# Kuntz-Lab/interactive-rate-tendons

Hardware: AMD Instinct MI355X
Metric: FK+collision checks/sec (3-tendon, 256^3 voxel env) (higher is better)
Workload: dtype f64

## Files before the change

include/tendon_hip.h:

```cpp
#ifndef TENDON_HIP_H
#define TENDON_HIP_H

#include <stddef.h>
#include <stdint.h>

#ifdef __cplusplus
extern "C" {
#endif

#define TR_MAX_TENDONS 8
#define TR_MAX_COEF    8

typedef enum {
  TR_OK                = 0,
  TR_ERR_INVALID_ARG   = 1,
  TR_ERR_OUT_OF_RANGE  = 2,
  TR_ERR_DOMAIN        = 3,
  TR_ERR_LENGTH        = 4,
  TR_ERR_RUNTIME       = 5,
  TR_ERR_HIP           = 6,
  TR_ERR_UNSUPPORTED   = 7
} tr_status;

typedef struct {
// ... 358 lines not shown
int tr_roadmap_state_query_profile(tr_roadmap *rm, double out[4]);

int tr_roadmap_ik_batch_loaded(tr_roadmap *rm, const tr_space_params *sp, const tr_tip_query_params *params, const tr_tip_connect_params *connect,
                               const tr_shoot_params *shoot, const tr_edge_loads *loads, const double *requests, int64_t n, double *controls,
                               double *tips, double *error, int32_t *neighbor_vertex, int32_t *ik_vertex, int32_t *outcome,
                               double *last_valid_t, double *vu0, int64_t *counts);
int tr_roadmap_solve_tips_loaded(tr_roadmap *rm, const tr_space_params *sp, const tr_tip_query_params *params, const tr_tip_connect_params *connect,
                                 const tr_shoot_params *shoot, const tr_edge_loads *loads, const int32_t *starts, const double *requests, int64_t n,
                                 int32_t n_threads, double *controls, double *tips, double *error, int32_t *neighbor_vertex, int32_t *ik_vertex,
                                 int32_t *outcome, double *last_valid_t, double *vu0, int64_t *counts, int32_t *status, double *cost,
                                 int64_t *path_offsets, tr_roadmap_stats *stats);
int tr_roadmap_set_tips_loaded(tr_roadmap *rm, const tr_shoot_params *shoot, const tr_edge_loads *loads, const uint64_t *present_bits);

int tr_knn_edges(tr_ctx *ctx, const double *states, int64_t n, int32_t k, double max_distance, int32_t *edges,
                 int64_t capacity, int64_t *n_edges);
int tr_knn_edges_dev(tr_ctx *ctx, const double *d_states, int64_t n, int32_t k, double max_distance, int32_t *d_edges,
                     int64_t capacity, int64_t *n_edges);
int tr_validate_edges_indexed_dev(tr_ctx *ctx, const tr_space_params *sp, const double *d_states, int64_t n_states,
                                  const int32_t *d_edges, int64_t n_edges, uint64_t *d_valid_bits, int32_t *d_n_fk,
                                  int64_t *n_domain_errors);
int tr_signature_words(const tr_ctx *ctx);
int tr_sample_valid_vertices_sig_dev(tr_ctx *ctx, uint64_t seed, uint64_t first_candidate, const double *lo, const double *hi,
                                     int64_t n_want, int64_t max_candidates, double *d_states, double *d_tips, int64_t *d_index,
                                     uint32_t *d_sig, int64_t *n_accepted, int64_t *n_tried, void *stream);
int tr_validate_candidates_sig_dev(tr_ctx *ctx, uint64_t seed, uint64_t first, int64_t count, const double *lo, const double *hi,
                                   uint64_t *d_valid_bits, double *d_tips, uint32_t *d_sig, void *stream);
int tr_validate_edges_indexed_sig_dev(tr_ctx *ctx, const tr_space_params *sp, const double *d_states, int64_t n_states,
                                      const uint32_t *d_vertex_sig, const int32_t *d_edges, int64_t n_edges,
                                      uint64_t *d_valid_bits, int32_t *d_n_fk, int64_t *n_domain_errors);

int tr_signature_packed_words(const tr_ctx *ctx);
int tr_pack_signatures_dev(tr_ctx *ctx, const uint32_t *d_sig, int64_t n_rows, uint32_t *d_packed, int64_t *n_uncodable, void *stream);
int tr_unpack_signatures_dev(tr_ctx *ctx, const uint32_t *d_packed, int64_t n_rows, uint32_t *d_sig, void *stream);

int tr_knn_range(tr_ctx *ctx, const double *states, int64_t n, int64_t first_query, int64_t n_queries, int32_t k,
                 double max_distance, int32_t *idx, double *dist);
int tr_knn_table_edges(tr_ctx *ctx, const int32_t *idx, int64_t n, int32_t k, int32_t *edges, int64_t capacity, int64_t *n_edges);
int tr_knn_range_dev(tr_ctx *ctx, const double *d_states, int64_t n, int64_t first_query, int64_t n_queries, int32_t k,
                     double max_distance, int32_t *d_idx);
int tr_knn_table_edges_dev(tr_ctx *ctx, const int32_t *d_idx, int64_t n, int32_t k, int32_t *d_edges, int64_t capacity,
                           int64_t *n_edges);

int tr_kstar_k(const tr_ctx *ctx, int64_t n_milestones);


#define TR_PROFILE_SLOTS 6
int tr_profile_begin(tr_ctx *ctx);
int tr_profile_read(tr_ctx *ctx, int64_t launches[TR_PROFILE_SLOTS], double total_ms[TR_PROFILE_SLOTS]);
int tr_profile_end(tr_ctx *ctx);

int tr_set_debug(tr_ctx *ctx, uint32_t bits);

int tr_edge_schedule_last(const tr_ctx *ctx, uint32_t stats[4]);


#ifdef __cplusplus
}
#endif
#endif
```

interactive-rate-tendons_amd/_lib.py:

```python
import ctypes as C
import os
import subprocess

_PKG = os.path.dirname(os.path.abspath(__file__))
_ROOT = os.path.dirname(_PKG)
LIB_PATH = os.environ.get("TENDON_HIP_LIB") or os.path.join(_PKG, "libtendon_hip.so")
SRC_DIR = os.path.join(_PKG, "csrc")
HEADER = os.path.join(_ROOT, "include", "tendon_hip.h")

TR_OK, TR_ERR_INVALID_ARG, TR_ERR_OUT_OF_RANGE, TR_ERR_DOMAIN, TR_ERR_LENGTH, TR_ERR_RUNTIME, \
    TR_ERR_HIP, TR_ERR_UNSUPPORTED = range(8)

TR_FLAG_CONVERGED, TR_FLAG_LENGTH_OK, TR_FLAG_NO_SELFCOL, TR_FLAG_NO_VOXCOL, TR_FLAG_DOMAIN = 1, 2, 4, 8, 16
TR_CHECKER_BACKBONE, TR_CHECKER_SPHERES = 0, 1
TR_PROFILE_SLOTS = 6
PROFILE_SLOT_NAMES = ("fk_rk4_batch", "backbone_voxel_sweep", "cached_blocks_vs_grid", "edge_helpers", "fk_sweep_fused", "fk_verdict")

ABI_SYMBOLS = (
    "tr_create", "tr_destroy", "tr_last_error", "tr_state_size", "tr_num_points", "tr_device",
    "tr_home_lengths", "tr_set_grid", "tr_set_checker", "tr_grid_add_spheres", "tr_grid_add_capsules", "tr_grid_remove_interior", "tr_grid_dilate",
    "tr_grid_dilate_sphere", "tr_get_grid", "tr_reserve", "tr_reserve_edges", "tr_fk_batch", "tr_fk_batch_dev", "tr_fk_batch_retraction_dev",
    "tr_validate_shapes_retraction_dev",
    "tr_validate_batch", "tr_validate_batch_dev", "tr_validate_shapes_dev", "tr_validate_edges", "tr_validate_edges_indexed", "tr_validate_edges_last_valid",
    "tr_validate_edges_discrete",
    "tr_check_cached", "tr_check_cached_dev", "tr_check_cached_subset_dev", "tr_state_layout", "tr_space_weights", "tr_kstar_k",
    "tr_roadmap_create", "tr_roadmap_destroy", "tr_roadmap_last_error", "tr_roadmap_set_caches", "tr_roadmap_set_caches_dev", "tr_roadmap_prepare", "tr_roadmap_clear_validity",
    "tr_roadmap_revalidate", "tr_roadmap_get_validity", "tr_roadmap_set_validity", "tr_roadmap_solve", "tr_roadmap_fetch_paths", "tr_roadmap_search_stats", "tr_roadmap_profile", "tr_roadmap_release_search_state", "tr_roadmap_reserve_search_state", "tr_roadmap_search_state_bytes", "tr_roadmap_search_sweeps", "tr_voxelize_batch", "tr_voxelize_edges", "tr_voxelize_edges_indexed", "tr_connect_edges_indexed", "tr_voxelize_fetch", "tr_voxelize_fetch_dev", "tr_voxelize_count", "tr_knn", "tr_knn_range", "tr_knn_table_edges", "tr_knn_edges", "tr_knn_edges_dev", "tr_knn_range_dev", "tr_knn_table_edges_dev", "tr_validate_edges_indexed_dev", "tr_signature_words", "tr_signature_packed_words", "tr_pack_signatures_dev", "tr_unpack_signatures_dev", "tr_validate_candidates_sig_dev", "tr_validate_edges_indexed_sig_dev", "tr_profile_begin", "tr_profile_read", "tr_profile_end",
    "tr_set_debug", "tr_edge_schedule_last",
    "tr_candidate_states", "tr_candidate_states_dev", "tr_validate_candidates_dev", "tr_compact_rows_dev",
    "tr_sample_valid_vertices", "tr_sample_valid_vertices_dev", "tr_sample_valid_vertices_sig_dev",
    "tr_fk_tips", "tr_fk_tips_dev", "tr_tip_jacobian", "tr_tip_jacobian_dev", "tr_ik_batch", "tr_ik_batch_dev",
    "tr_roadmap_set_tips", "tr_roadmap_nearest_tips", "tr_roadmap_nearest_tips_dev", "tr_roadmap_ik_batch", "tr_roadmap_solve_tips",
    "tr_roadmap_tip_query_profile",
    "tr_roadmap_nearest_states", "tr_roadmap_nearest_states_dev", "tr_roadmap_ik_batch_connect", "tr_roadmap_solve_tips_connect",
    "tr_roadmap_tip_connect_stats",
    "tr_fk_loaded_batch", "tr_fk_loaded_batch_dev", "tr_fk_loaded_batch_retraction_dev", "tr_set_loaded_retraction",
    "tr_validate_edges_loaded", "tr_validate_edges_loaded_indexed", "tr_edges_loaded_vertex_strains", "tr_edges_loaded_last",
    "tr_sample_valid_vertices_loaded", "tr_sample_valid_vertices_loaded_dev", "tr_voxelize_batch_loaded",
    "tr_voxelize_edges_loaded_indexed", "tr_connect_edges_loaded_indexed",
    "tr_ik_loaded_batch", "tr_ik_loaded_batch_dev",
    "tr_tip_jacobian_loaded", "tr_tip_jacobian_loaded_dev",
    "tr_fk_loaded_tips", "tr_fk_loaded_tips_dev",
    "tr_roadmap_ik_batch_loaded", "tr_roadmap_solve_tips_loaded", "tr_roadmap_set_tips_loaded",
    "tr_set_load_profile", "tr_clear_load_profile", "tr_get_load_profile",
    "tr_roadmap_attach_states", "tr_roadmap_attach_states_dev", "tr_roadmap_solve_seeded", "tr_roadmap_solve_states",
    "tr_roadmap_state_query_profile",
)


class TrRobotDesc(C.Structure):
    _fields_ = [
        ("r", C.c_double),
        ("L", C.c_double), ("dL", C.c_double), ("ro", C.c_double), ("ri", C.c_double),
        ("E", C.c_double), ("nu", C.c_double),
        ("n_tendons", C.c_int32), ("n_a", C.c_int32), ("n_m", C.c_int32),
        ("C", C.POINTER(C.c_double)), ("D", C.POINTER(C.c_double)),
        ("max_tension", C.POINTER(C.c_double)), ("min_length", C.POINTER(C.c_double)),
        ("max_length", C.POINTER(C.c_double)),
        ("enable_rotation", C.c_int32), ("enable_retraction", C.c_int32),
        ("residual_threshold", C.c_double),
    ]


class TrSpaceParams(C.Structure):
    _fields_ = [("min_tension_change", C.c_double), ("min_rotation_change", C.c_double),
                ("min_retraction_change", C.c_double)]


class TrIkParams(C.Structure):
    _fields_ = [("max_iters", C.c_int32), ("mu_init", C.c_double), ("stop_threshold_JT_err_inf", C.c_double),
                ("stop_threshold_Dp", C.c_double), ("stop_threshold_err", C.c_double), ("finite_difference_delta", C.c_double)]


class TrShootParams(C.Structure):
    _fields_ = [("max_iters", C.c_int32), ("mu_init", C.c_double), ("stop_threshold_JT_err_inf", C.c_double),
                ("stop_threshold_Dp", C.c_double), ("finite_difference_delta", C.c_double)]


TR_LOAD_FRAME_BASE, TR_LOAD_FRAME_WORLD = 0, 1


# ... 276 lines not shown
    L.tr_fk_loaded_batch_dev.argtypes = [vp, shp, vp, i64, i64, vp, i64, vp, i64, vp, vp, vp, vp, vp, vp, vp, vp, vp, vp, vp, vp, vp, vp, P(i64), vp]
    L.tr_set_loaded_retraction.argtypes = [vp, C.c_int]
    L.tr_fk_loaded_batch_retraction_dev.argtypes = [vp, shp, vp, i64, i64, vp, i64, vp, i64, vp, vp, vp, vp, vp, vp, vp, vp, vp, vp, vp, vp, vp, vp, vp, P(i64), vp]
    elp = P(TrEdgeLoads)
    L.tr_validate_edges_loaded.argtypes = [vp, P(TrSpaceParams), shp, elp, dp, dp, i64, P(C.c_uint64), dp, i32p, P(i64), P(i64), P(i64)]
    L.tr_validate_edges_loaded_indexed.argtypes = [vp, P(TrSpaceParams), shp, elp, dp, i64, i32p, i64, P(C.c_uint64), i32p, P(i64), P(i64), P(i64)]
    L.tr_edges_loaded_vertex_strains.argtypes = [vp, i64, dp]
    L.tr_edges_loaded_last.argtypes = [vp, P(i64)]
    L.tr_sample_valid_vertices_loaded.argtypes = [vp, shp, elp, u64, u64, dp, dp, i64, i64, dp, dp, P(i64), dp, P(i64), P(i64), P(i64), P(i64)]
    L.tr_sample_valid_vertices_loaded_dev.argtypes = [vp, shp, elp, u64, u64, dp, dp, i64, i64, vp, vp, vp, vp, P(i64), P(i64), P(i64), P(i64), vp]
    L.tr_voxelize_batch_loaded.argtypes = [vp, shp, elp, dp, i64, P(i64), P(C.c_uint64), dp, P(i64), P(i64)]
    L.tr_voxelize_edges_loaded_indexed.argtypes = [vp, P(TrSpaceParams), shp, elp, dp, i64, i32p, i64, P(i64), P(C.c_uint64), i32p, P(i64), P(i64)]
    L.tr_connect_edges_loaded_indexed.argtypes = L.tr_voxelize_edges_loaded_indexed.argtypes
    L.tr_ik_loaded_batch.argtypes = [vp, P(TrIkParams), shp, elp, dp, i64, dp, i64, dp, dp, dp, dp, dp, dp, i32p, i32p, dp, P(C.c_uint8), P(i64)]
    L.tr_ik_loaded_batch_dev.argtypes = [vp, P(TrIkParams), shp, elp, vp, i64, vp, i64, dp, dp, vp, vp, vp, vp, vp, vp, vp, vp, P(i64), vp]
    L.tr_tip_jacobian_loaded.argtypes = [vp, shp, elp, dp, i64, C.c_double, dp, dp, dp, dp, dp, dp, P(C.c_uint8), dp, P(i64), P(i64)]
    L.tr_tip_jacobian_loaded_dev.argtypes = [vp, shp, elp, vp, i64, C.c_double, vp, vp, vp, vp, vp, vp, vp, vp, vp, P(i64), vp]
    tqp = P(TrTipQueryParams)
    L.tr_roadmap_set_tips.argtypes = [vp, dp, P(u64)]
    L.tr_roadmap_nearest_tips.argtypes = [vp, dp, i64, C.c_int32, i32p, dp]
    L.tr_roadmap_nearest_tips_dev.argtypes = [vp, vp, i64, C.c_int32, vp, vp]
    L.tr_roadmap_ik_batch.argtypes = [vp, P(TrSpaceParams), tqp, dp, i64, dp, dp, dp, i32p, i32p, dp]
    L.tr_roadmap_solve_tips.argtypes = [vp, P(TrSpaceParams), tqp, i32p, dp, i64, C.c_int32, dp, dp, dp, i32p, i32p, dp, i32p, dp, P(i64),
                                        P(TrRoadmapStats)]
    L.tr_roadmap_tip_query_profile.argtypes = [vp, dp]
    tcp = P(TrTipConnectParams)
    L.tr_roadmap_nearest_states.argtypes = [vp, dp, i64, C.c_int32, C.c_double, i32p, dp]
    L.tr_roadmap_nearest_states_dev.argtypes = [vp, vp, i64, C.c_int32, C.c_double, vp, vp]
    L.tr_roadmap_ik_batch_connect.argtypes = [vp, P(TrSpaceParams), tqp, tcp, dp, i64, dp, dp, dp, i32p, i32p, i32p, dp]
    L.tr_roadmap_solve_tips_connect.argtypes = [vp, P(TrSpaceParams), tqp, tcp, i32p, dp, i64, C.c_int32, dp, dp, dp, i32p, i32p, i32p, dp, i32p,
                                                dp, P(i64), P(TrRoadmapStats)]
    L.tr_roadmap_tip_connect_stats.argtypes = [vp, P(i64)]
    L.tr_fk_loaded_tips.argtypes = [vp, shp, dp, i64, dp, i64, dp, i64, dp, dp, P(C.c_uint8), dp, P(i64)]
    L.tr_fk_loaded_tips_dev.argtypes = [vp, shp, vp, i64, vp, i64, vp, i64, vp, vp, vp, vp, P(i64), vp]
    L.tr_roadmap_ik_batch_loaded.argtypes = [vp, P(TrSpaceParams), tqp, tcp, shp, elp, dp, i64, dp, dp, dp, i32p, i32p, i32p, dp, dp, P(i64)]
    L.tr_roadmap_solve_tips_loaded.argtypes = [vp, P(TrSpaceParams), tqp, tcp, shp, elp, i32p, dp, i64, C.c_int32, dp, dp, dp, i32p, i32p, i32p,
                                               dp, dp, P(i64), i32p, dp, P(i64), P(TrRoadmapStats)]
    L.tr_roadmap_set_tips_loaded.argtypes = [vp, shp, elp, P(u64)]
    atp, u8p = P(TrAttachParams), P(C.c_uint8)
    L.tr_roadmap_attach_states.argtypes = [vp, P(TrSpaceParams), atp, C.c_int32, dp, i64, u8p, i32p, dp, u8p, i32p, P(i64)]
    L.tr_roadmap_attach_states_dev.argtypes = [vp, P(TrSpaceParams), atp, C.c_int32, vp, i64, vp, vp, vp, vp, vp, P(i64)]
    L.tr_roadmap_solve_seeded.argtypes = [vp, i64, P(i64), i32p, dp, P(i64), i32p, dp, dp, C.c_int32, i32p, dp, i32p, i32p, P(i64), P(TrRoadmapStats)]
    L.tr_roadmap_solve_states.argtypes = [vp, P(TrSpaceParams), atp, dp, dp, i64, C.c_int32, i32p, dp, i32p, i32p, u8p, i32p, i32p, P(i64),
                                          P(TrRoadmapStats)]
    L.tr_roadmap_state_query_profile.argtypes = [vp, dp]
    L.tr_set_load_profile.argtypes = [vp, i64, dp, dp]
    L.tr_clear_load_profile.argtypes = [vp]
    L.tr_get_load_profile.argtypes = [vp, dp, i64, P(i64)]
    L.tr_profile_begin.argtypes = [vp]
    L.tr_profile_read.argtypes = [vp, P(i64), dp]
    L.tr_profile_end.argtypes = [vp]
    L.tr_set_debug.argtypes = [vp, C.c_uint32]
    L.tr_edge_schedule_last.argtypes = [vp, P(C.c_uint32)]
    _lib = L
    return L


def check(ctx, status):
    if status == TR_OK:
        return
    msg = lib().tr_last_error(ctx)
    msg = msg.decode() if msg else "status %d" % status
    raise _EXC.get(status, TendonHipError)(msg)
```

interactive-rate-tendons_amd/csrc/edge_queue_kernel.hpp:

```cpp
#pragma once
#include "verdict_kernel.hpp"
#define TRK_EDGE_DEVICE_ONLY
#include "edge_kernel.hpp"

namespace trk {

__device__ __forceinline__ uint32_t eq_load(const uint32_t *p) { return __hip_atomic_load(p, __ATOMIC_RELAXED, __HIP_MEMORY_SCOPE_AGENT); }
__device__ __forceinline__ void eq_wait_vm() { asm volatile("s_waitcnt vmcnt(0)" ::: "memory"); }
__device__ __forceinline__ void eq_release() {
  eq_wait_vm();
  __builtin_amdgcn_fence(__ATOMIC_RELEASE, "agent");
  eq_wait_vm();
}
__device__ __forceinline__ void eq_acquire() {
  __builtin_amdgcn_fence(__ATOMIC_ACQUIRE, "agent");
  eq_wait_vm();
}
__device__ __forceinline__ int eq_bcast(int v) { return __builtin_amdgcn_readfirstlane(v); }
struct EqClock {
  unsigned long long t;
  __device__ __forceinline__ void start() { t = wall_clock64(); }
  __device__ __forceinline__ void lap(uint32_t *ctl, int word) {
    const unsigned long long n = wall_clock64();
    if (threadIdx.x == 0) __hip_atomic_fetch_add((unsigned long long *)(ctl + word), n - t, __ATOMIC_RELAXED, __HIP_MEMORY_SCOPE_AGENT);
// ... 77 lines not shown
    if (n > 0) { pos = eq_bcast(r_pos); return true; }
    d = (uint32_t)eq_bcast((int)d); t = (uint32_t)eq_bcast((int)t);
    if (d + t != seen) { seen = d + t; idle = 0; }
    else if (++idle > (1u << 19)) {
      if (lane == 0) __hip_atomic_fetch_or(ctl + EQ_FLAGS, EQF_STUCK, __ATOMIC_RELAXED, __HIP_MEMORY_SCOPE_AGENT);
      return false;
    }
    __builtin_amdgcn_s_sleep(127);
    if (idle > 16) __builtin_amdgcn_s_sleep(127);
    if (idle > 256) { __builtin_amdgcn_s_sleep(127); __builtin_amdgcn_s_sleep(127); }
  }
}

template <int N, bool ROT, class Form = TableRouting>
__global__ __launch_bounds__(64, (N <= TRK_VERDICT_TWO_WAVE_MAXN ? 2 : 1)) void fk_edge_queue(
    RobotK K, const double *__restrict__ tab, const StepK *__restrict__ steps, int nsteps,
    const VerdictArgs *__restrict__ va, const EdgeQueueArgs *__restrict__ qa, const FusedSweepArgs *__restrict__ sa) {
  const int lane = threadIdx.x;
  EqClock clk;
  clk.start();
#ifdef TRK_EQ_TRACE
  int tr_round = 0;
#endif
  for (;;) {
    int zero = 0;
    asm volatile("" : "+s"(zero));
    const EdgeQueueArgs &q = qa[zero];
    int h = 0, cnt = 0;
    if (!eq_claim(q, h, cnt)) break;
    clk.lap(q.ctl, EQ_T_CLAIM);
    const bool live = lane < cnt;
    const int slot = h + lane;
    int e_lane = -1;
    {
      bool bail = false;
      if (live) {
        const uint32_t *flag = (const uint32_t *)q.sample_edge + slot;
        unsigned spins = 0;
        while ((e_lane = (int)eq_load(flag)) < 0) {
          if (eq_load(q.ctl + EQ_FLAGS) != 0u) { bail = true; break; }
          if (++spins > (1u << 22)) {
            __hip_atomic_fetch_or(q.ctl + EQ_FLAGS, EQF_STUCK, __ATOMIC_RELAXED, __HIP_MEMORY_SCOPE_AGENT);
            bail = true; break;
          }
          __builtin_amdgcn_s_sleep(8);
        }
      }
      if (__any(bail)) break;
    }
    eq_acquire();
    clk.lap(q.ctl, EQ_T_READY);

    PointSweep<false, true> ps;
    ps.va = va;
    ps.dn_prev = 0.0f; ps.sph_state = 0u;
    ps.qhead = 0; ps.qcount = 0; ps.active = false;
    ps.P = va->P; ps.CH = va->CH; ps.NM = va->NM; ps.Kl = (ps.P - 1 + ps.CH - 1) / ps.CH; ps.ms_next = 0; ps.ms_k = 0;
    ps.sigst.init(); ps.sig_row_of = -1; ps.sig_first_row = 0; ps.sig_row0 = h; ps.sig_cnt = cnt;
    __syncthreads();
    VL_U(VLay<true>::HIT + lane) = 0u; VL_U(VLay<true>::INPREV + lane) = 0u; VL_F(VLay<true>::DIST + lane) = 0.0f;
    __syncthreads();
    const int S = K.state_size;
    const double *st_eff = q.states + ((int64_t)h - (int64_t)blockIdx.x * 64) * S;
    const int64_t n_eff = (int64_t)blockIdx.x * 64 + cnt;
    {
      const int sb = eq_stash_base(ps.NM);
      VL_I(sb + lane) = e_lane;
      if (lane == 0) { VL_I(sb + 64) = h; VL_I(sb + 65) = cnt; VL_U(sb + 66) = (uint32_t)clk.t; VL_U(sb + 67) = (uint32_t)(clk.t >> 32); }
    }
    FkLane<N> fl_;
    {
      FkOut out{nullptr, nullptr, nullptr, nullptr, nullptr, nullptr, nullptr, nullptr, nullptr, nullptr};
      fk_uniform_body<N, ROT, false, false, Form>(st_eff, n_eff, 0, K, tab, steps, nsteps, out, ps, nullptr, &fl_);
    }
    ps.template sig_finish<false>();
    ps.finish();
    while (ps.qcount > 0) ps.flush();
    __syncthreads();
    LaneVerdict lv;
    int e2, h2, cnt2;
    {
      const VerdictArgs a = *va;
      const int sb = eq_stash_base(a.NM);
      e2 = VL_I(sb + lane); h2 = VL_I(sb + 64); cnt2 = VL_I(sb + 65);
      clk.t = (unsigned long long)VL_U(sb + 66) | ((unsigned long long)VL_U(sb + 67) << 32);
      lv = verdict_decide<N, false, true>(a, fl_, lane < cnt2);
    }
    const bool live2 = lane < cnt2;
    int zero2 = 0;
    asm volatile("" : "+s"(zero2));
    const EdgeQueueArgs &q2 = qa[zero2];
#ifdef TRK_EQ_TRACE
    const uint32_t tr_start = (uint32_t)clk.t;
    const unsigned long long tr_w0 = wall_clock64(), tr_c0 = (unsigned long long)clock64();
    { float x = (float)lane; for (int i = 0; i < 2000; i++) x = __builtin_fmaf(x, 1.0000001f, 0.5f); if (x == 12345.678f) asm volatile("s_nop 0"); }
    const unsigned long long tr_w1 = wall_clock64(), tr_c1 = (unsigned long long)clock64();
    const uint32_t tr_mhz = tr_w1 > tr_w0 ? (uint32_t)((tr_c1 - tr_c0) * 100ull / (tr_w1 - tr_w0)) : 0u;
#endif
    clk.lap(q2.ctl, EQ_T_FK);
#ifdef TRK_EQ_TRACE
    const uint32_t tr_fk = (uint32_t)clk.t;
#endif
    if (__any(lv.pending)) {
      __syncthreads();
      const double *st2 = q2.states + ((int64_t)h2 - (int64_t)blockIdx.x * 64) * K.state_size;
      const int64_t n2 = (int64_t)blockIdx.x * 64 + cnt2;
      fk_uniform_body<N, ROT, false, false, Form>(st2, n2, q2.fb_ld, K, tab, steps, nsteps, q2.fb_out, NoPointHook(), nullptr, nullptr);
      __syncthreads();
      const FusedSweepArgs fa = *sa;
      bool exact = false;
      sweep_body<false>(q2.fb_in, n2, q2.fb_ld, fa.P, fa.CH, fa.NM, K, fa.g, fa.grid, fa.near_grid, 1, fa.debug, nullptr, nullptr, nullptr, &exact);
      __syncthreads();
      const uint32_t npend = (uint32_t)__popcll(__ballot(lv.pending));
// ... 167 lines not shown
```

interactive-rate-tendons_amd/csrc/fk_inst.hip:

```cpp
#include "fk_launch.hpp"
#include "fk_kernel.hpp"
#if TRK_INST_KIND == 1
#include "fk_retract_kernel.hpp"
#elif TRK_INST_KIND == 2
#include "fused_kernel.hpp"
#elif TRK_INST_KIND == 3
#include "verdict_kernel.hpp"
#elif TRK_INST_KIND == 4
#define TRK_WITH_RETRACT_VERDICT
#include "fk_retract_kernel.hpp"
#include "verdict_kernel.hpp"
#elif TRK_INST_KIND == 5
#include "edge_queue_kernel.hpp"
#elif TRK_INST_KIND == 6 || TRK_INST_KIND == 7
#define TRK_LOADED_WITH_INTEGRATOR
#include "fk_loaded_kernel.hpp"
#elif TRK_INST_KIND == 8
#include "fk_loaded_retract_kernel.hpp"
#endif

namespace trk {

using HelixForm = std::conditional_t<(TRK_INST_N <= TRK_K1_TWO_WAVE_MAXN), UniformHelix, TableRouting>;
[[maybe_unused]] static bool helix_form(const RobotK &K) { return TRK_INST_N <= TRK_K1_TWO_WAVE_MAXN && K.routing_form == TRK_ROUTING_HELIX; }
// ... 44 lines not shown
static void go(const FkLaunch &a, const LoadedIn &in) {
  const unsigned grid = (unsigned)((a.n + 63) / 64);
  hipLaunchKernelGGL((fk_loaded_profile<TRK_INST_N, ROT, WR>), dim3(grid), dim3(64), 0, a.stream, a.d_states, a.n, a.ld, a.K,
                     a.d_tab, a.d_steps, a.n_steps, a.out, in);
}
template <> void launch_fk_loaded_profile<TRK_INST_N>(const FkLaunch &a, const LoadedIn &in) {
  if (a.rotation) { if (a.write_R) go<true, true>(a, in); else go<true, false>(a, in); }
  else            { if (a.write_R) go<false, true>(a, in); else go<false, false>(a, in); }
}
#elif TRK_INST_KIND == 8
template <bool ROT, bool WR>
static void go(const FkLaunch &a, const LoadedIn &in) {
  const unsigned grid = (unsigned)((a.n + 63) / 64);
  hipLaunchKernelGGL((fk_loaded_retract<TRK_INST_N, ROT, WR>), dim3(grid), dim3(64), 0, a.stream, a.d_states, a.n, a.ld, a.K, a.d_poly,
                     a.d_tab, a.d_steps, a.n_steps, a.k_first, a.d_tgrid, a.d_hl, a.out, in);
}
template <> void launch_fk_loaded_retract<TRK_INST_N>(const FkLaunch &a, const LoadedIn &in) {
  if (a.rotation) { if (a.write_R) go<true, true>(a, in); else go<true, false>(a, in); }
  else            { if (a.write_R) go<false, true>(a, in); else go<false, false>(a, in); }
}
template <> void launch_shoot_start_retract<TRK_INST_N>(const FkLaunch &a, const double *guess, double *vu) {
  const unsigned grid = (unsigned)((a.n + 63) / 64);
  hipLaunchKernelGGL((shoot_start_retract<TRK_INST_N>), dim3(grid), dim3(64), 0, a.stream, a.d_states, a.n, a.K, a.d_poly, guess, vu);
}
#elif TRK_INST_KIND == 4
template <bool ROT, bool SPH, bool SIG>
static void go(const FkLaunch &a, const VerdictArgs *va, size_t lds) {
  const unsigned grid = (unsigned)((a.n + 63) / 64);
  const RetractHandoff ho{a.d_handoff, a.handoff_ld};
  hipLaunchKernelGGL((fk_retract_prologue<TRK_INST_N, ROT>), dim3(grid), dim3(64), 0, a.stream, a.d_states, a.n, a.K, a.d_poly, a.d_tab, a.d_steps,
                     a.n_steps, a.k_first, a.d_tgrid, a.d_hl, a.d_perm, ho);
  hipLaunchKernelGGL((fk_verdict_retract<TRK_INST_N, ROT, SPH, SIG>), dim3(grid), dim3(64), lds, a.stream, a.d_states, a.n, a.K, a.d_poly,
                     a.d_tab, a.d_steps, a.n_steps, a.k_first, a.d_tgrid, a.d_hl, a.out.tips, va, ho);
}
template <bool SPH, bool SIG>
static void go_rot(const FkLaunch &a, const VerdictArgs *va, size_t lds) {
  if (a.rotation) go<true, SPH, SIG>(a, va, lds); else go<false, SPH, SIG>(a, va, lds);
}
template <> void launch_fk_verdict_retract<TRK_INST_N>(const FkLaunch &a, const VerdictArgs *va, size_t lds, bool spheres, bool with_sig) {
  if (spheres) { if (with_sig) go_rot<true, true>(a, va, lds); else go_rot<true, false>(a, va, lds); }
  else         { if (with_sig) go_rot<false, true>(a, va, lds); else go_rot<false, false>(a, va, lds); }
}
template <bool ROT>
static void go_list(const FkLaunch &a, const FusedSweepArgs *sweep, size_t lds, const int32_t *list, const uint32_t *count) {
  const unsigned grid = (unsigned)((a.n + 63) / 64);
  hipLaunchKernelGGL((fk_sweep_retract_list<TRK_INST_N, ROT>), dim3(grid), dim3(64), lds, a.stream, a.d_states, a.n, a.ld, a.K,
                     a.d_poly, a.d_tab, a.d_steps, a.n_steps, a.k_first, a.d_tgrid, a.d_hl, a.out, sweep, list, count);
}
template <> void launch_fk_sweep_retract_list<TRK_INST_N>(const FkLaunch &a, const FusedSweepArgs *sweep, size_t lds, const int32_t *list,
                                                          const uint32_t *count) {
  if (a.rotation) go_list<true>(a, sweep, lds, list, count); else go_list<false>(a, sweep, lds, list, count);
}
#elif TRK_INST_KIND == 3
template <bool ROT, bool SPH, bool SIG, class Form>
static void go(const FkLaunch &a, const VerdictArgs *va, size_t lds) {
  const unsigned grid = (unsigned)((a.n + 63) / 64);
  hipLaunchKernelGGL((fk_verdict<TRK_INST_N, ROT, SPH, SIG, Form>), dim3(grid), dim3(64), lds, a.stream, a.d_states, a.n, a.K, a.d_tab, a.d_steps,
                     a.n_steps, a.out.tips, va);
}
template <bool SPH, bool SIG>
static void go_rot(const FkLaunch &a, const VerdictArgs *va, size_t lds) {
  if (helix_form(a.K)) { if (a.rotation) go<true, SPH, SIG, HelixForm>(a, va, lds); else go<false, SPH, SIG, HelixForm>(a, va, lds); }
  else                 { if (a.rotation) go<true, SPH, SIG, TableRouting>(a, va, lds); else go<false, SPH, SIG, TableRouting>(a, va, lds); }
}
template <> void launch_fk_verdict<TRK_INST_N>(const FkLaunch &a, const VerdictArgs *va, size_t lds, bool spheres, bool with_sig) {
  if (spheres) { if (with_sig) go_rot<true, true>(a, va, lds); else go_rot<true, false>(a, va, lds); }
  else         { if (with_sig) go_rot<false, true>(a, va, lds); else go_rot<false, false>(a, va, lds); }
}
#elif TRK_INST_KIND == 2
template <bool ROT, class Form>
static void go_list(const FkLaunch &a, const FusedSweepArgs *sweep, size_t lds, const int32_t *list, const uint32_t *count) {
  const unsigned grid = (unsigned)((a.n + 63) / 64);
  hipLaunchKernelGGL((fk_sweep_fused_list<TRK_INST_N, ROT, Form>), dim3(grid), dim3(64), lds, a.stream, a.d_states, a.n, a.ld, a.K,
                     a.d_tab, a.d_steps, a.n_steps, a.out, sweep, list, count);
}
template <> void launch_fk_sweep_fused_list<TRK_INST_N>(const FkLaunch &a, const FusedSweepArgs *sweep, size_t lds, const int32_t *list,
                                                        const uint32_t *count) {
  if (helix_form(a.K)) { if (a.rotation) go_list<true, HelixForm>(a, sweep, lds, list, count); else go_list<false, HelixForm>(a, sweep, lds, list, count); }
  else                 { if (a.rotation) go_list<true, TableRouting>(a, sweep, lds, list, count); else go_list<false, TableRouting>(a, sweep, lds, list, count); }
}
template <bool ROT, class Form>
static void go(const FkLaunch &a, const FusedSweepArgs *sweep, size_t lds) {
  const unsigned grid = (unsigned)((a.n + 63) / 64);
  hipLaunchKernelGGL((fk_sweep_fused<TRK_INST_N, ROT, Form>), dim3(grid), dim3(64), lds, a.stream, a.d_states, a.n, a.ld, a.K,
                     a.d_tab, a.d_steps, a.n_steps, a.out, sweep);
}
template <> void launch_fk_sweep_fused<TRK_INST_N>(const FkLaunch &a, const FusedSweepArgs *sweep, size_t lds) {
  if (helix_form(a.K)) { if (a.rotation) go<true, HelixForm>(a, sweep, lds); else go<false, HelixForm>(a, sweep, lds); }
  else                 { if (a.rotation) go<true, TableRouting>(a, sweep, lds); else go<false, TableRouting>(a, sweep, lds); }
}
#else
#if TRK_INST_KIND == 1
template <bool ROT, bool WR>
static void go(const FkLaunch &a) {
  const unsigned grid = (unsigned)((a.n + 63) / 64);
  hipLaunchKernelGGL((fk_rk4_batch_retract<TRK_INST_N, ROT, WR>), dim3(grid), dim3(64), 0, a.stream, a.d_states, a.n, a.ld, a.K,
                     a.d_poly, a.d_tab, a.d_steps, a.n_steps, a.k_first, a.d_tgrid, a.d_hl, a.out, a.d_perm, a.d_wave_k_begin);
}
template <> void launch_fk_retract<TRK_INST_N>(const FkLaunch &a) {
#else
template <bool ROT, bool WR>
static void go(const FkLaunch &a) {
  const unsigned grid = (unsigned)((a.n + 63) / 64);
  if (helix_form(a.K))
    hipLaunchKernelGGL((fk_rk4_batch_uniform<TRK_INST_N, ROT, WR, HelixForm>), dim3(grid), dim3(64), 0, a.stream, a.d_states, a.n, a.ld, a.K,
                       a.d_tab, a.d_steps, a.n_steps, a.out);
  else
    hipLaunchKernelGGL((fk_rk4_batch_uniform<TRK_INST_N, ROT, WR>), dim3(grid), dim3(64), 0, a.stream, a.d_states, a.n, a.ld, a.K,
                       a.d_tab, a.d_steps, a.n_steps, a.out);
}
template <> void launch_fk_uniform<TRK_INST_N>(const FkLaunch &a) {
#endif
  if (a.rotation) { if (a.write_R) go<true, true>(a); else go<true, false>(a); }
  else            { if (a.write_R) go<false, true>(a); else go<false, false>(a); }
}
#endif

}
```

interactive-rate-tendons_amd/csrc/fk_kernel.hpp:

```cpp
#pragma once
#include <type_traits>
#include <hip/hip_runtime.h>
#include "tr_types.hpp"

namespace trk {

#ifndef TRK_NEWTON_STEPS
#define TRK_NEWTON_STEPS 1
#endif
__device__ __forceinline__ double fast_rcp(double x) {
  double y = __builtin_amdgcn_rcp(x);
  double e = __builtin_fma(-x, y, 1.0);
  y = __builtin_fma(e, y, y);
#if TRK_NEWTON_STEPS > 1
  e = __builtin_fma(-x, y, 1.0);
  y = __builtin_fma(e, y, y);
#endif
  return y;
}
__device__ __forceinline__ double fast_rsqrt(double x) {
  double y = __builtin_amdgcn_rsq(x);
  double hx = 0.5 * x;
  double t = __builtin_fma(-hx * y, y, 0.5);
  y = __builtin_fma(y, t, y);
// ... 281 lines not shown
#pragma clang fp contract(fast)
  const double hh = h * 0.5;
  const double b1 = h * (1.0 / 6.0), b2 = h * (1.0 / 3.0);
  double aR[9], av[3], au[3];
#pragma unroll
  for (int q = 0; q < 3; q++) { av[q] = v[q]; au[q] = u[q]; }
  double sR[9], sv[3], su[3], qs[3], qm[3];
#pragma unroll
  for (int q = 0; q < 9; q++) sR[q] = R[q];
#pragma unroll
  for (int q = 0; q < 3; q++) { sv[q] = v[q]; su[q] = u[q]; }
#pragma unroll
  for (int st = 0; st < 4; st++) {
    double ts = (st == 0) ? t : ((st == 3) ? t + h : t + hh);
    asm volatile("" : "+v"(ts) : "v"(sv[0]), "v"(su[0]));
    const double bw = (st == 0 || st == 3) ? b1 : b2;
    const double aw = (st == 2) ? h : hh;
    double dv[3], du[3], sd[N];
    strain_rates_routed<N>(sv, su, tau, [&](int j, double (&r6)[6]) { route(ts, j, r6); }, K, dv, du, sd, stage_load(sR));
    position_quadrature(st, sR, sv, b1, qs, qm, p);
    {
      const double v2 = __builtin_fma(sv[2], sv[2], __builtin_fma(sv[1], sv[1], sv[0] * sv[0]));
      Lb += bw * (v2 * fast_rsqrt(v2));
    }
#pragma unroll
    for (int j = 0; j < N; j++) Li[j] += bw * sd[j];
    double dR[9];
    frame_rate(st, sR, su, dR, aR);
#pragma unroll
    for (int q = 0; q < 3; q++) { av[q] += bw * dv[q]; au[q] += bw * du[q]; }
    if (st < 3) {
#pragma unroll
      for (int q = 0; q < 9; q++) sR[q] = R[q] + aw * dR[q];
#pragma unroll
      for (int q = 0; q < 3; q++) { sv[q] = v[q] + aw * dv[q]; su[q] = u[q] + aw * du[q]; }
    }
  }
#pragma unroll
  for (int q = 0; q < 9; q++) R[q] = __builtin_fma(b1, aR[q], R[q]);
#pragma unroll
  for (int q = 0; q < 3; q++) { v[q] = av[q]; u[q] = au[q]; }
}


template <int N>
struct FkLane {
  bool converged;
  double Li[N];
  double tip[3];
};

struct NoPointHook {
  __device__ __forceinline__ void begin(bool) const {}
  __device__ __forceinline__ void operator()(int, double, double, double) const {}
  __device__ __forceinline__ void tip_point(int, bool, bool, double, double, double, bool = true) const {}
};

template <class H, class = void> struct HookLiInLds { static constexpr int from = 1 << 30; };
template <class H> struct HookLiInLds<H, std::void_t<decltype(H::kLiInLdsFrom)>> { static constexpr int from = H::kLiInLdsFrom; };
template <class OnPoint> __host__ __device__ constexpr bool li_in_lds(int N) {
  return N >= HookLiInLds<std::remove_cv_t<std::remove_reference_t<OnPoint>>>::from && N <= 4;
}

template <int N, bool ROT, bool WRITE_R, bool WANT_L = true, class Form = TableRouting, class OnPoint = NoPointHook>
__device__ __forceinline__ void fk_uniform_body(
    const double *__restrict__ states, int64_t n, int64_t ld, const RobotK &K,
    const double *__restrict__ tab, const StepK *__restrict__ steps, int nsteps, const FkOut &out,
    OnPoint &&on_point = NoPointHook(), const int32_t *__restrict__ row_map = nullptr, FkLane<N> *lane_out = nullptr) {
#pragma clang fp contract(fast)
  const int64_t i = (int64_t)blockIdx.x * 64 + threadIdx.x;
  const bool live = i < n;
  const int64_t il = live ? i : (n - 1);
  const int64_t ic = row_map ? (int64_t)row_map[il] : il;
  const int S = K.state_size;
  double tau[N];
#pragma unroll
  for (int j = 0; j < N; j++) tau[j] = states[ic * S + j];
  constexpr bool kLiLds = li_in_lds<OnPoint>(N);
  double *li_lds = nullptr;
  if constexpr (kLiLds) {
    __shared__ double li_lds_store[N * 64];
    li_lds = li_lds_store;
#pragma unroll
    for (int j = 0; j < N; j++) li_lds[j * 64 + threadIdx.x] = 0.0;
  }
  double rc = 1.0, rs = 0.0, r22 = 1.0;
  if (ROT) {
    const double th = states[ic * S + N];
    rs = sin(th); rc = cos(th);
    r22 = (1.0 - rc) + rc;
  }

  double v[3], u[3];
  bool conv;
  initial_bending<N>(tau, tab, K, v, u, conv);
  on_point.begin(conv && live);

  double R[9] = {1, 0, 0, 0, 1, 0, 0, 0, 1};
  double p[3] = {0, 0, 0};
  double Lb = 0;
  double Li[N];
#pragma unroll
  for (int j = 0; j < N; j++) Li[j] = 0;

  auto store_point = [&](int j) {
    const int64_t o = (int64_t)j * ld + i;
    double x = p[0], y = p[1], z = p[2];
    if (ROT) { const double x2 = __builtin_fma(rc, x, -(rs * y)), y2 = __builtin_fma(rs, x, rc * y); x = x2; y = y2; z = r22 * z; }
    on_point(j, x, y, z);
    if (!live) return;
    if (out.px) { out.px[o] = x; out.py[o] = y; out.pz[o] = z; }
    if (WRITE_R) {
      const int64_t PS = (int64_t)K.n_points * ld;
#pragma unroll
      for (int c = 0; c < 3; c++) {
        double a = R[c * 3 + 0], b = R[c * 3 + 1], cc = R[c * 3 + 2];
        if (ROT) { const double a2 = rc * a - rs * b, b2 = rs * a + rc * b; a = a2; b = b2; cc = r22 * cc; }
        out.R[(c * 3 + 0) * PS + o] = a; out.R[(c * 3 + 1) * PS + o] = b; out.R[(c * 3 + 2) * PS + o] = cc;
      }
    }
  };
  store_point(0);

  for (int k = 0; k < nsteps; k++) {
    const double h = steps[k].h;
    const int obs = steps[k].obs;
    const double *__restrict__ rt = tab + (size_t)(1 + 3 * k) * (N * 6);
    const double hh = h * 0.5;
    const double b1 = h * (1.0 / 6.0), b2 = h * (1.0 / 3.0);
    double aR[9], av[3], au[3];
#pragma unroll
    for (int q = 0; q < 3; q++) { av[q] = v[q]; au[q] = u[q]; }
    double sR[9], sv[3], su[3];
    double qs[3], qm[3];
#pragma unroll
    for (int q = 0; q < 9; q++) sR[q] = R[q];
#pragma unroll
    for (int q = 0; q < 3; q++) { sv[q] = v[q]; su[q] = u[q]; }

#pragma unroll
    for (int st = 0; st < 4; st++) {
      const double *__restrict__ ri = rt + (st == 0 ? 0 : (st == 3 ? 2 : 1)) * (N * 6);
      const double bw = (st == 0 || st == 3) ? b1 : b2;
      const double aw = (st == 2) ? h : hh;
      double dv[3], du[3], sd[N];
      strain_rates<N, NoLoad, Form>(sv, su, tau, ri, K, dv, du, sd);
      position_quadrature(st, sR, sv, b1, qs, qm, p);
      if (WANT_L && out.L) {
        const double v2 = __builtin_fma(sv[2], sv[2], __builtin_fma(sv[1], sv[1], sv[0] * sv[0]));
        Lb += bw * (v2 * fast_rsqrt(v2));
      }
      if constexpr (kLiLds) {
#pragma unroll
        for (int j = 0; j < N; j++) li_lds[j * 64 + threadIdx.x] += bw * sd[j];
      } else {
#pragma unroll
        for (int j = 0; j < N; j++) Li[j] += bw * sd[j];
      }
      double dR[9];
      frame_rate(st, sR, su, dR, aR);
#pragma unroll
      for (int q = 0; q < 3; q++) { av[q] += bw * dv[q]; au[q] += bw * du[q]; }
      if (st < 3) {
#pragma unroll
        for (int q = 0; q < 9; q++) sR[q] = R[q] + aw * dR[q];
#pragma unroll
        for (int q = 0; q < 3; q++) { sv[q] = v[q] + aw * dv[q]; su[q] = u[q] + aw * du[q]; }
      }
    }
#pragma unroll
    for (int q = 0; q < 9; q++) R[q] = __builtin_fma(b1, aR[q], R[q]);
#pragma unroll
    for (int q = 0; q < 3; q++) { v[q] = av[q]; u[q] = au[q]; }
    if (obs >= 0) store_point(obs);
  }

  if constexpr (kLiLds) {
#pragma unroll
    for (int j = 0; j < N; j++) Li[j] = li_lds[j * 64 + threadIdx.x];
  }
  if (live) {
    if (out.L) out.L[i] = Lb;
    if (out.Li) {
#pragma unroll
      for (int j = 0; j < N; j++) out.Li[(int64_t)j * ld + i] = Li[j];
    }
    if (out.converged) out.converged[i] = conv ? 1 : 0;
    if (out.n_points) out.n_points[i] = K.n_points;
    if (out.tips) {
      double x = p[0], y = p[1], z = p[2];
      if (ROT) { const double x2 = __builtin_fma(rc, x, -(rs * y)), y2 = __builtin_fma(rs, x, rc * y); x = x2; y = y2; z = r22 * z; }
      out.tips[3 * i + 0] = x; out.tips[3 * i + 1] = y; out.tips[3 * i + 2] = z;
    }
  }
  if (lane_out) {
    lane_out->converged = conv;
#pragma unroll
    for (int j = 0; j < N; j++) lane_out->Li[j] = Li[j];
    double x = p[0], y = p[1], z = p[2];
    if (ROT) { const double x2 = __builtin_fma(rc, x, -(rs * y)), y2 = __builtin_fma(rs, x, rc * y); x = x2; y = y2; z = r22 * z; }
    lane_out->tip[0] = x; lane_out->tip[1] = y; lane_out->tip[2] = z;
  }
}

template <int N, bool ROT, bool WRITE_R, class Form = TableRouting>
__global__ __launch_bounds__(64, (N <= TRK_K1_TWO_WAVE_MAXN ? 2 : 1)) void fk_rk4_batch_uniform(
    const double *__restrict__ states, int64_t n, int64_t ld, RobotK K,
    const double *__restrict__ tab, const StepK *__restrict__ steps, int nsteps, FkOut out) {
  fk_uniform_body<N, ROT, WRITE_R, true, Form>(states, n, ld, K, tab, steps, nsteps, out);
}

}
```

interactive-rate-tendons_amd/csrc/fk_launch.hpp:

```cpp
#pragma once
#include <hip/hip_runtime.h>
#include "tr_types.hpp"

namespace trk {

struct FkLaunch {
  const double *d_states; int64_t n, ld;
  RobotK K;
  bool rotation, write_R;
  const double *d_tab; const StepK *d_steps; int n_steps;
  const PolyK *d_poly; int k_first; const double *d_tgrid, *d_hl;
  FkOut out;
  hipStream_t stream;
  double *d_handoff = nullptr; int64_t handoff_ld = 0; const int32_t *d_perm = nullptr;
  const int32_t *d_wave_k_begin = nullptr;
};

struct LoadedIn {
  const double *wrench; int64_t wrench_ld;
  const double *dist; int64_t dist_ld;
  const double *vu;
  const int32_t *list;
  int32_t Q;
  const double *tip_route;
  double *res; int64_t ldr;
  double *vu_tip;
  const double *weights = nullptr;
};

struct FusedSweepArgs;
struct VerdictArgs;
struct EdgeQueueArgs;
template <int N> void launch_fk_uniform(const FkLaunch &a);
template <int N> void launch_fk_sweep_fused(const FkLaunch &a, const FusedSweepArgs *sweep, size_t lds);
template <int N> void launch_fk_sweep_fused_list(const FkLaunch &a, const FusedSweepArgs *sweep, size_t lds, const int32_t *list,
                                                 const uint32_t *count);
template <int N> void launch_fk_verdict(const FkLaunch &a, const VerdictArgs *va, size_t lds, bool spheres, bool with_sig);
template <int N> void launch_fk_retract(const FkLaunch &a);
template <int N> void launch_fk_verdict_retract(const FkLaunch &a, const VerdictArgs *va, size_t lds, bool spheres, bool with_sig);
template <int N> void launch_fk_sweep_retract_list(const FkLaunch &a, const FusedSweepArgs *sweep, size_t lds, const int32_t *list,
                                                   const uint32_t *count);

template <int N> void launch_fk_edge_queue(const FkLaunch &a, const VerdictArgs *va, size_t lds, const EdgeQueueArgs *qa,
                                           const FusedSweepArgs *sweep, unsigned waves);
template <int N> int fk_edge_queue_waves_per_cu(const RobotK &K, size_t lds);

template <int N> void launch_fk_loaded(const FkLaunch &a, const LoadedIn &in);
template <int N> void launch_fk_loaded_profile(const FkLaunch &a, const LoadedIn &in);
template <int N> void launch_shoot_start(const FkLaunch &a, const double *guess, double *vu);
template <int N> void launch_fk_loaded_retract(const FkLaunch &a, const LoadedIn &in);
template <int N> void launch_shoot_start_retract(const FkLaunch &a, const double *guess, double *vu);

#define TRK_DECL_FK(N) template <> void launch_fk_uniform<N>(const FkLaunch &); template <> void launch_fk_retract<N>(const FkLaunch &); \
  template <> void launch_fk_loaded<N>(const FkLaunch &, const LoadedIn &); template <> void launch_fk_loaded_profile<N>(const FkLaunch &, const LoadedIn &); \
  template <> void launch_shoot_start<N>(const FkLaunch &, const double *, double *); \
  template <> void launch_fk_loaded_retract<N>(const FkLaunch &, const LoadedIn &); \
  template <> void launch_shoot_start_retract<N>(const FkLaunch &, const double *, double *); \
  template <> void launch_fk_sweep_fused<N>(const FkLaunch &, const FusedSweepArgs *, size_t); \
  template <> void launch_fk_sweep_fused_list<N>(const FkLaunch &, const FusedSweepArgs *, size_t, const int32_t *, const uint32_t *); \
  template <> void launch_fk_verdict<N>(const FkLaunch &, const VerdictArgs *, size_t, bool, bool); \
  template <> void launch_fk_verdict_retract<N>(const FkLaunch &, const VerdictArgs *, size_t, bool, bool); \
  template <> void launch_fk_sweep_retract_list<N>(const FkLaunch &, const FusedSweepArgs *, size_t, const int32_t *, const uint32_t *); \
  template <> void launch_fk_edge_queue<N>(const FkLaunch &, const VerdictArgs *, size_t, const EdgeQueueArgs *, const FusedSweepArgs *, unsigned); \
  template <> int fk_edge_queue_waves_per_cu<N>(const RobotK &, size_t);
TRK_DECL_FK(1) TRK_DECL_FK(2) TRK_DECL_FK(3) TRK_DECL_FK(4) TRK_DECL_FK(5) TRK_DECL_FK(6) TRK_DECL_FK(7) TRK_DECL_FK(8)
#undef TRK_DECL_FK

}
```

interactive-rate-tendons_amd/csrc/sweep_kernel.hpp:

```cpp
#pragma once
#include <hip/hip_runtime.h>
#include "tr_types.hpp"

#ifndef TRK_K2_PF
#define TRK_K2_PF 4
#endif

namespace trk {

struct V3 { double x, y, z; };

__device__ __forceinline__ double dot3(const V3 &a, const V3 &b) {
#pragma clang fp contract(off)
  return a.x * b.x + a.y * b.y + a.z * b.z;
}

__device__ __forceinline__ bool segment_aabox_intersect(const V3 &A, const V3 &B, const GridK &g) {
#pragma clang fp contract(off)
  const V3 AB = {B.x - A.x, B.y - A.y, B.z - A.z};
  const double len = sqrt(dot3(AB, AB)) / 2;
  const V3 U = {AB.x / (2 * len), AB.y / (2 * len), AB.z / (2 * len)};
  const V3 Ua = {fabs(U.x), fabs(U.y), fabs(U.z)};
  const V3 P = {(A.x + B.x) / 2 - (g.xmax + g.xmin) / 2, (A.y + B.y) / 2 - (g.ymax + g.ymin) / 2,
                (A.z + B.z) / 2 - (g.zmax + g.zmin) / 2};
// ... 201 lines not shown
  const double tx = A.x - g.xmin, ty = A.y - g.ymin, tz = A.z - g.zmin;
  const double qx = tx * g.inv_dx, qy = ty * g.inv_dy, qz = tz * g.inv_dz;
  int cx = (int)qx, cy = (int)qy, cz = (int)qz;
  const double fx = qx - (double)cx, fy = qy - (double)cy, fz = qz - (double)cz;
  const double lo = 1e-9, hi = 1.0 - 1e-9;
  if (!(fx > lo && fx < hi && fy > lo && fy < hi && fz > lo && fz < hi)) {
    cx = (int)(long)(tx / g.dx); cy = (int)(long)(ty / g.dy); cz = (int)(long)(tz / g.dz);
  }
  return ((uint32_t)cx & 1023u) | (((uint32_t)cy & 1023u) << 10) | (((uint32_t)cz & 1023u) << 20);
}

#ifndef TRK_SIG_FLUSH_UNROLL
#define TRK_SIG_FLUSH_UNROLL 1
#endif
constexpr int SIG_T = 8, SIG_LDS_STRIDE = 72, SIG_LDS_WORDS = SIG_T * SIG_LDS_STRIDE;
struct SigStage {
  int cur, mask;
  __device__ __forceinline__ void init() { cur = -1; mask = 0; }
  template <class Word>
  __device__ __forceinline__ void flush(Word &&W, uint32_t *__restrict__ sig, int64_t stride, int row_of, int first_row) {
    if (cur < 0) return;
    __syncthreads();
    const int lane = threadIdx.x, w = lane & (SIG_T - 1), sub = lane >> 3;
    const int j = cur * SIG_T + w;
#pragma unroll TRK_SIG_FLUSH_UNROLL
    for (int it = 0; it < 8; it++) {
      const int r = it * 8 + sub;
      const int ro = __shfl(row_of, r, 64), fr = __shfl(first_row, r, 64);
      const uint32_t v = W(w * SIG_LDS_STRIDE + r);
      if (((mask >> w) & 1) && ro >= 0 && j >= fr) sig[(int64_t)ro * stride + j] = v;
    }
    __syncthreads();
    cur = -1; mask = 0;
  }
  template <class Word>
  __device__ __forceinline__ void put(Word &&W, uint32_t *__restrict__ sig, int64_t stride, int row_of, int first_row, int row, bool on,
                                      uint32_t value) {
    const int tile = row >> 3;
    if (tile != cur) { flush(W, sig, stride, row_of, first_row); cur = tile; }
    if (on) W((row & (SIG_T - 1)) * SIG_LDS_STRIDE + (int)threadIdx.x) = value;
    mask |= 1 << (row & (SIG_T - 1));
  }
};

struct SignatureHook {
  static constexpr int kLiInLdsFrom = 3;
  const FusedSweepArgs *sa;
  int64_t n;
  bool any;
  SigStage st;
  __device__ __forceinline__ static uint32_t &word(int i) { extern __shared__ float lds[]; return ((uint32_t *)lds)[i]; }
  __device__ __forceinline__ int row_of() const { const int64_t i = (int64_t)blockIdx.x * 64 + threadIdx.x; return i < n ? (int)i : -1; }
  __device__ __forceinline__ void begin(bool) const {}
  __device__ __forceinline__ void operator()(int j, double x, double y, double z) {
    if (!any) return;
    int zero = 0;
    asm volatile("" : "+s"(zero));
    const FusedSweepArgs &a = sa[zero];
    st.put([](int i) -> uint32_t & { return word(i); }, a.sig, a.sig_stride, row_of(), 0, j, true, cell_signature(x, y, z, a.g));
  }
  __device__ __forceinline__ void finish() {
    if (!any) return;
    st.flush([](int i) -> uint32_t & { return word(i); }, sa->sig, sa->sig_stride, row_of(), 0);
  }
};

__device__ __forceinline__ bool exact_self_collision(const SweepIn &in, int64_t ic, int64_t ld, int P, int np,
                                                     bool act, double hmax, double r, bool brute) {
#pragma clang fp contract(off)
  const double consider = 3.0 * r;
  const double rsum = r + r;
  const double h_eff = hmax * (1.0 + 1e-9) + 1e-300;
  const double inv_h = 1.0 / h_eff;
  bool selfhit = false;
  act = act && np > 2;
  for (int a = 0; a < P - 3; ++a) {
    if (!__any(act && a < np - 3)) break;
    const bool act_a = act && a < np - 3;
    const int64_t oa = (int64_t)a * ld + ic;
    V3 pa = {0, 0, 0}, pa1 = {0, 0, 0};
    double acc_a1 = 0;
    if (act_a) {
      pa = V3{in.px[oa], in.py[oa], in.pz[oa]};
      pa1 = V3{in.px[oa + ld], in.py[oa + ld], in.pz[oa + ld]};
      acc_a1 = in.acc[oa + ld];
    }
    int b = a + 2;
    while (b < P - 1) {
      const bool act_b = act_a && !selfhit && b < np - 1;
      if (!__any(act_b)) break;
      int skip = 0x7fffffff;
      if (act_b) {
        const int64_t ob = (int64_t)b * ld + ic;
        const V3 pb = {in.px[ob], in.py[ob], in.pz[ob]};
        skip = 1;
        bool need_exact = true;
        if (!brute) {
          const V3 d = {pa.x - pb.x, pa.y - pb.y, pa.z - pb.z};
          const double D = sqrt(dot3(d, d));
          const double slack = D - rsum - 2.0 * h_eff - 1e-9 * (1.0 + D);
          if (slack > 0.0) {
            need_exact = false;
            const double m = slack * inv_h * (1.0 - 1e-9);
            skip = m > 1.0 ? (m < 1e6 ? (int)m : 1000000) : 1;
          }
        }
        if (need_exact) {
// ... 411 lines not shown
```

interactive-rate-tendons_amd/csrc/tendon_hip.hip:

```cpp
#include <hip/hip_runtime.h>
#include <sched.h>

#include <algorithm>
#include <cfloat>
#include <cmath>
#include <cstdio>
#include <cstdlib>
#include <cstring>
#include <functional>
#include <initializer_list>
#include <chrono>
#include <thread>
#include <ctime>
#include <limits>
#include <mutex>
#include <string>
#include <vector>

#include "../../include/tendon_hip.h"
#include "tr_types.hpp"
#include "fk_launch.hpp"
#include "fk_lin_launch.hpp"
#include "sweep_kernel.hpp"
#include "sphere_kernel.hpp"
// ... 73 lines not shown
    for (T **f : fields) if (const int rc = alloc(c, f, count)) return rc;
    return 0;
  }
  void release() {
    for (void *q : held) (void)hipFree(q);
    held.clear();
  }
};

struct RoundCount {
  tr_ctx *c = nullptr;
  uint32_t *d = nullptr, *h = nullptr;
  int reserve(tr_ctx *ctx, DevOwner &own);
  int zero(int slot, hipStream_t s);
  int read(int slot, hipStream_t s, int64_t &active);
  void release() { if (h) (void)hipHostFree(h); d = h = nullptr; }
};

}

struct tr_ctx {
  std::recursive_mutex mu;
  int device = 0;
  std::string err;
  RobotK K{};
  std::vector<double> C, D, max_tension;
  std::vector<double> t;
  std::vector<StepK> steps;
  std::vector<double> step_t;
  double *d_tab = nullptr;
  StepK *d_steps = nullptr;
  PolyK *d_poly = nullptr;
  double *d_tgrid = nullptr;
  double *d_hl = nullptr;
  int k_first = 0;
  bool has_grid = false;
  GridK G{};
  uint64_t *d_grid = nullptr;
  uint64_t *d_near = nullptr;
  uint32_t n_blocks = 0;
  int checker = TR_CHECKER_BACKBONE;
  float *d_sph_near = nullptr, *d_sph_tmp = nullptr;
  bool sph_near_valid = false;
  uint64_t *d_envw[2] = {nullptr, nullptr};
  uint32_t envw_blocks = 0;
  Workspace ws;
  EdgeDev edge;
  trk::MergeScratch merge;
  int64_t max_chunk = 1 << 20;
  int64_t edge_pool_max = 1 << 22;
  int64_t edge_slots_max = 1 << 24;
  int64_t edge_slots_now = 0;
  double ch_scale = 2.0;
  int64_t k1_round = 1 << 17;
  int fuse = 2;
  int64_t fb_cap = 1 << 17;
  struct RetractOrder {
    uint32_t *keys[2] = {nullptr, nullptr}; int32_t *vals[2] = {nullptr, nullptr}; int64_t cap = 0;
    int32_t *kbegin = nullptr;
    double *handoff = nullptr; int64_t handoff_cap = 0;
    trk::MergeScratch ms;
  };
  static constexpr int kMaxLanes = edge_plan::kMaxLanes;
  struct EdgeLaneDev {
    hipStream_t stream = nullptr;
    uint32_t *hc = nullptr;
    uint32_t *counters = nullptr;
    int32_t *fb_list = nullptr; uint32_t *fb_count = nullptr; int64_t fb_list_cap = 0;
    RetractOrder ro;
  } lane[kMaxLanes];
  int edge_lanes = kMaxLanes;
  bool edge_lanes_fixed = false;
  bool edge_kernels_loaded = false;
  bool edge_queue = true;
  bool edge_queue_forced = false;
  int edge_queue_waves = 0;
  uint32_t edge_queue_last[4] = {0, 0, 0, 0};
  double edge_rate_seen = 0.0;
  bool edge_lane_guess_forced = false;
  double edge_lane_guess = 6.0;
  int64_t retract_sort_min = kRetractSortMin;
  bool rows_one_step = false;
  bool retract_wave_start = true;
  struct VerdictRing {
    static constexpr int kSlots = 16;
    trk::VerdictArgs *d_slots = nullptr, *h_slots = nullptr;
    hipEvent_t ev[kSlots];
    bool used[kSlots] = {};
    int next = 0;
  } vring;
  struct FusedRing {
    static constexpr int kSlots = 16;
    trk::FusedSweepArgs *d_slots = nullptr, *h_slots = nullptr;
    hipEvent_t ev[kSlots];
    bool used[kSlots] = {};
    int next = 0;
  } fused;
  struct KnnScratch { void *p[13] = {}; size_t cap[13] = {}; } knn;
  struct VoxStore { uint32_t *ids = nullptr; uint64_t *masks = nullptr; int64_t cap = 0, n = 0; } vstore;
  uint32_t *d_vids = nullptr; uint64_t *d_vmasks = nullptr; int32_t *d_vcounts = nullptr;
  uint64_t *d_vbits = nullptr;
  int64_t vox_cap = 0;
  int32_t *d_item_src = nullptr, *d_item_edge = nullptr; int64_t vox_items_cap = 0;
  struct Pipe {
    bool ready = false;
    int64_t chunk = 0;
// ... 514 lines not shown
  a.P = ctx->K.n_points; a.debug = ctx->debug;
  a.g = ctx->G; a.grid = ctx->d_grid; a.near_grid = ctx->d_near; a.valid_bits = d_bits; a.flags = d_flags;
  {
    const GridK &g = ctx->G;
    a.box[0] = g.xmin + 1e-6 * (g.xmax - g.xmin); a.box[1] = g.xmax - 1e-6 * (g.xmax - g.xmin);
    a.box[2] = g.ymin + 1e-6 * (g.ymax - g.ymin); a.box[3] = g.ymax - 1e-6 * (g.ymax - g.ymin);
    a.box[4] = g.zmin + 1e-6 * (g.zmax - g.zmin); a.box[5] = g.zmax - 1e-6 * (g.zmax - g.zmin);
  }
  a.fb_list = fb_list; a.fb_count = fb_count;
  a.sig = sig; a.sig_stride = sig_stride; a.np_out = np_out;
  a.radius = ctx->K.radius;
  for (int j = 0; j < TRK_MAX_TENDONS; j++) { a.home_Li[j] = ctx->K.home_Li[j]; a.min_len[j] = ctx->K.min_len[j]; a.max_len[j] = ctx->K.max_len[j]; }
  if (spheres) {
    a.field = ctx->d_sph_near; a.radius = ctx->K.radius;
    a.r_lo = (float)ctx->K.radius - 2e-6f; a.r_hi = (float)ctx->K.radius + 2e-6f;
  }
  if (ctx->K.enable_retraction && ctx->retract_sort_min > 0 && n >= ctx->retract_sort_min) {
    tr_ctx::RetractOrder &ro = ctx->lane[lane].ro;
    if ((rc = ensure_lane_order(ctx, lane, round_up(n, 64)))) return rc;
    const hipError_t e = trk::retraction_order(order_scratch(ctx, lane), d_states, n, ctx->K.state_size, ctx->K.L, ro.keys, ro.vals, &a.perm, s,
                                               ctx->K.dL, ctx->k_first, ctx->rows_one_step, ro.kbegin);
    a.wave_k_begin = ctx->retract_wave_start ? ro.kbegin : nullptr;
    if (e != hipSuccess) return fail(ctx, TR_ERR_HIP, std::string("retraction order: ") + hipGetErrorString(e));
    HIP_TRY(ctx, hipMemsetAsync(d_bits, 0, (size_t)((n + 63) / 64) * sizeof(uint64_t), s));
  }
  a.finish_hot();
  HIP_TRY(ctx, hipMemcpyAsync(vr.d_slots + vslot, &a, sizeof(a), hipMemcpyHostToDevice, s));
  HIP_TRY(ctx, hipMemsetAsync(fb_count, 0, sizeof(uint32_t), s));
  const bool ret = ctx->K.enable_retraction;
  const trk::FusedSweepArgs *d_fargs; size_t lds_f; int fslot;
  if ((rc = fused_args_slot(ctx, ws_sweep_in(ctx, fcol), spheres ? 2 : 1, d_bits, d_flags, s, &d_fargs, &lds_f, &fslot))) return rc;
  const trk::FkOut vout{nullptr, nullptr, nullptr, nullptr, nullptr, nullptr, d_tips, nullptr, nullptr, nullptr};
  trk::FkLaunch vl{d_states, n, 0, ctx->K, (bool)ctx->K.enable_rotation, false, ctx->d_tab, ctx->d_steps,
                   (int)ctx->steps.size(), ctx->d_poly, ctx->k_first, ctx->d_tgrid, ctx->d_hl, vout, s};
  if (ctx->K.enable_retraction) {
    tr_ctx::RetractOrder &ro = ctx->lane[lane].ro;
    const int64_t hld = round_up(n, 64);
    if (ro.handoff_cap < hld) {
      HIP_TRY(ctx, hipDeviceSynchronize());
      const int64_t want = hld + hld / 8;
      if ((rc = dev_alloc(ctx, &ro.handoff, (size_t)want * (19 + 2 * TRK_MAX_TENDONS + 3)))) return rc;
      ro.handoff_cap = want;
    }
    vl.d_handoff = ro.handoff; vl.handoff_ld = hld; vl.d_perm = a.perm;
  }
  const trk::FkOut fout = ws_fk_out(ctx, fcol);
  const trk::FkLaunch fl{d_states, cap, w.ld, ctx->K, (bool)ctx->K.enable_rotation, false, ctx->d_tab, ctx->d_steps,
                         (int)ctx->steps.size(), ctx->d_poly, ctx->k_first, ctx->d_tgrid, ctx->d_hl, fout, s};
  const size_t lds_v = trk::verdict_lds_bytes(a.NM, sig != nullptr);
  {
    ProfScope ps(ctx, 5, s);
    switch (ctx->K.n_tendons) {
#define TRK_CASE(N) case N: if (ret) trk::launch_fk_verdict_retract<N>(vl, vr.d_slots + vslot, lds_v, spheres, sig != nullptr); \
                            else trk::launch_fk_verdict<N>(vl, vr.d_slots + vslot, lds_v, spheres, sig != nullptr); break;
      TRK_CASE(1) TRK_CASE(2) TRK_CASE(3) TRK_CASE(4) TRK_CASE(5) TRK_CASE(6) TRK_CASE(7) TRK_CASE(8)
#undef TRK_CASE
      default: return fail(ctx, TR_ERR_OUT_OF_RANGE, "n_tendons out of range");
    }
    HIP_TRY(ctx, hipGetLastError());
  }
  {
    ProfScope ps(ctx, 4, s);
    switch (ctx->K.n_tendons) {
#define TRK_CASE(N) case N: if (ret) trk::launch_fk_sweep_retract_list<N>(fl, d_fargs, lds_f, fb_list, fb_count); \
                            else trk::launch_fk_sweep_fused_list<N>(fl, d_fargs, lds_f, fb_list, fb_count); break;
      TRK_CASE(1) TRK_CASE(2) TRK_CASE(3) TRK_CASE(4) TRK_CASE(5) TRK_CASE(6) TRK_CASE(7) TRK_CASE(8)
#undef TRK_CASE
      default: break;
    }
    HIP_TRY(ctx, hipGetLastError());
  }
  HIP_TRY(ctx, hipEventRecord(vr.ev[vslot], s));
  vr.used[vslot] = true;
  HIP_TRY(ctx, hipEventRecord(ctx->fused.ev[fslot], s));
  ctx->fused.used[fslot] = true;
  return TR_OK;
}

int launch_edge_queue(tr_ctx *ctx, hipStream_t s, uint32_t *sig, int64_t sig_stride, const trk::EdgeQueueArgs *qa, unsigned waves) {
  if (!ctx->has_grid) return fail(ctx, TR_ERR_INVALID_ARG, "no obstacle grid set (tr_set_grid)");
  Workspace &w = ctx->ws;
  if (w.ld < (int64_t)waves * 64) return fail(ctx, TR_ERR_RUNTIME, "edge queue: workspace smaller than the launch");
  tr_ctx::VerdictRing &vr = ctx->vring;
  if (!vr.d_slots) {
    HIP_TRY(ctx, hipMalloc((void **)&vr.d_slots, sizeof(trk::VerdictArgs) * tr_ctx::VerdictRing::kSlots));
    HIP_TRY(ctx, hipHostMalloc((void **)&vr.h_slots, sizeof(trk::VerdictArgs) * tr_ctx::VerdictRing::kSlots, hipHostMallocDefault));
    for (auto &e : vr.ev) HIP_TRY(ctx, hipEventCreateWithFlags(&e, hipEventDisableTiming));
  }
  const int vslot = vr.next;
  vr.next = (vr.next + 1) % tr_ctx::VerdictRing::kSlots;
  if (vr.used[vslot]) HIP_TRY(ctx, hipEventSynchronize(vr.ev[vslot]));
  trk::VerdictArgs &a = vr.h_slots[vslot];
  a = trk::VerdictArgs{};
  size_t lds_k2;
  sweep_geometry(ctx, a.CH, a.NM, lds_k2);
  a.P = ctx->K.n_points; a.debug = ctx->debug;
  a.g = ctx->G; a.grid = ctx->d_grid; a.near_grid = ctx->d_near;
  {
    const GridK &g = ctx->G;
    a.box[0] = g.xmin + 1e-6 * (g.xmax - g.xmin); a.box[1] = g.xmax - 1e-6 * (g.xmax - g.xmin);
    a.box[2] = g.ymin + 1e-6 * (g.ymax - g.ymin); a.box[3] = g.ymax - 1e-6 * (g.ymax - g.ymin);
    a.box[4] = g.zmin + 1e-6 * (g.zmax - g.zmin); a.box[5] = g.zmax - 1e-6 * (g.zmax - g.zmin);
  }
  a.sig = sig; a.sig_stride = sig_stride;
  a.radius = ctx->K.radius;
  for (int j = 0; j < TRK_MAX_TENDONS; j++) { a.home_Li[j] = ctx->K.home_Li[j]; a.min_len[j] = ctx->K.min_len[j]; a.max_len[j] = ctx->K.max_len[j]; }
  a.finish_hot();
// ... 126 lines not shown
  if (const char *e = std::getenv("TENDON_HIP_EDGE_QUEUE_WAVES")) { const int v = std::atoi(e); if (v >= 1 && v <= 8192) c->edge_queue_waves = v; }
  if (const char *e = std::getenv("TENDON_HIP_EDGE_LANE_GUESS")) { const double v = std::atof(e); if (v >= 0.5 && v <= 64.0) { c->edge_lane_guess = v; c->edge_lane_guess_forced = true; } }
  if (const char *e = std::getenv("TENDON_HIP_EDGE_POOL")) {
    const long long v = std::atoll(e);
    if (v >= 256 && v <= (1ll << 24)) c->edge_pool_max = c->edge_slots_max = (int64_t)round_up(v, 64);
  }
  if (const char *e = std::getenv("TENDON_HIP_SHOOT_CHUNK")) { const long long v = std::atoll(e); if (v >= 1 && v <= (1ll << 20)) c->shoot_chunk = (int64_t)v; }
  if (const char *e = std::getenv("TENDON_HIP_LOADED_VERTEX_BATCH")) { const long long v = std::atoll(e); if (v >= 64 && v <= (1ll << 20)) c->loaded_vertex_batch = (int64_t)round_up(v, 64); }
  if (hipSetDevice(device) != hipSuccess) { delete c; return fail(nullptr, TR_ERR_HIP, "hipSetDevice failed"); }
  {
    int cus = 0;
    if (hipDeviceGetAttribute(&cus, hipDeviceAttributeMultiprocessorCount, device) == hipSuccess && cus > 0)
      c->k1_round = (int64_t)cus * 4 * (rb->n_tendons <= TRK_K1_TWO_WAVE_MAXN ? 2 : 1) * 64;
    c->fb_cap = c->k1_round;
  }
  if (const char *e = std::getenv("TENDON_HIP_FB_CAP")) { const long long v = std::atoll(e); if (v >= 64 && v <= (1ll << 20)) c->fb_cap = (int64_t)round_up(v, 64); }

  RobotK &K = c->K;
  const int N = rb->n_tendons;
  K.n_tendons = N; K.n_a = rb->n_a; K.n_m = rb->n_m;
  K.enable_rotation = rb->enable_rotation ? 1 : 0;
  K.enable_retraction = rb->enable_retraction ? 1 : 0;
  K.state_size = N + K.enable_rotation + K.enable_retraction;
  K.residual_threshold = rb->residual_threshold;
  K.radius = rb->r; K.L = rb->L; K.dL = rb->dL;
  c->C.assign(rb->C, rb->C + (size_t)N * rb->n_a);
  c->D.assign(rb->D, rb->D + (size_t)N * rb->n_m);
  c->max_tension.assign(rb->max_tension, rb->max_tension + N);
  for (int j = 0; j < N; j++) { K.min_len[j] = rb->min_length[j]; K.max_len[j] = rb->max_length[j]; }
  {
    const routing_form::Form rf = routing_form::classify(routing_spec(c), routing_env, TRK_K1_TWO_WAVE_MAXN);
    K.routing_form = rf.form; K.helix_omega = rf.omega; K.helix_rho2 = rf.rho * rf.rho;
  }
  {
    const double ro2 = rb->ro * rb->ro, ri2 = rb->ri * rb->ri;
    const double I = (1.0 / 4.0) * M_PI * (ro2 * ro2 - ri2 * ri2);
    const double Ar = M_PI * (ro2 - ri2);
    const double J = 2 * I;
    const double Gmod = rb->E / (2 * (1 + rb->nu));
    K.kb0 = rb->E * I; K.kb2 = J * Gmod; K.dkb = K.kb2 - K.kb0;
    K.ikb0 = 1 / (rb->E * I); K.ikb2 = 1 / (J * Gmod);
    K.ks0 = Gmod * Ar; K.ks2 = rb->E * Ar;
    K.iks0 = 1 / (Gmod * Ar); K.iks2 = 1 / (rb->E * Ar);
  }
  c->t = t_range(0.0, rb->L, rb->dL);
  K.n_points = (int)c->t.size();
  std::vector<double> &step_t = c->step_t;
  for (size_t j = 0; j + 1 < c->t.size(); j++) {
    double cur = c->t[j];
    const double tn = c->t[j + 1];
    bool any = false;
    while (tn - cur > DBL_EPSILON) {
      const double h = std::min(rb->dL, tn - cur);
      c->steps.push_back(StepK{h, -1, 0});
      step_t.push_back(cur);
      cur += h;
      any = true;
    }
    if (!any) { c->steps.push_back(StepK{0.0, -1, 0}); step_t.push_back(cur); }
    c->steps.back().obs = (int)j + 1;
  }
  const size_t ent = (size_t)N * 6;
  std::vector<double> tab((1 + 3 * c->steps.size()) * ent);
  routing_at(c, 0.0, tab.data());
  for (size_t k = 0; k < c->steps.size(); k++) {
    const double tk = step_t[k], h = c->steps[k].h;
    routing_at(c, tk, &tab[(1 + 3 * k + 0) * ent]);
    routing_at(c, tk + h * 0.5, &tab[(1 + 3 * k + 1) * ent]);
    routing_at(c, tk + h, &tab[(1 + 3 * k + 2) * ent]);
  }
  home_lengths(c, c->t, 0.0, K.home_Li);
  for (size_t k = 0; k < c->steps.size(); k++) if (c->steps[k].obs == 1) c->k_first = (int)k + 1;
  c->rows_one_step = (int)c->steps.size() - c->k_first == K.n_points - 2;
  for (size_t k = (size_t)c->k_first; k < c->steps.size() && c->rows_one_step; k++)
    if (c->steps[k].obs != (int)k - c->k_first + 2) c->rows_one_step = false;
  std::vector<double> hl(c->t.size() * (size_t)N);
  for (size_t q = 0; q < c->t.size(); q++)
    for (int j = 0; j < N; j++) {
      const double *Cj = &c->C[(size_t)j * rb->n_a], *Dj = &c->D[(size_t)j * rb->n_m];
      double Cdot[TRK_MAX_COEF] = {0}, Ddot[TRK_MAX_COEF] = {0};
      for (int k = 1; k < rb->n_a; k++) Cdot[k - 1] = k * Cj[k];
      for (int k = 1; k < rb->n_m; k++) Ddot[k - 1] = k * Dj[k];
      const double dd = poly_at(Ddot, rb->n_m, c->t[q]), dv = poly_at(Dj, rb->n_m, c->t[q]), cd = poly_at(Cdot, rb->n_a, c->t[q]);
      hl[q * N + j] = std::sqrt(dd * dd + (dv * dv) * (cd * cd) + 1);
    }
  PolyK poly{};
  for (int j = 0; j < N; j++) {
    for (int i = 0; i < rb->n_a; i++) poly.C[j][i] = c->C[(size_t)j * rb->n_a + i];
    for (int i = 0; i < rb->n_m; i++) poly.D[j][i] = c->D[(size_t)j * rb->n_m + i];
    const int rdeg = poly_degree(&c->D[(size_t)j * rb->n_m], rb->n_m), tdeg = poly_degree(&c->C[(size_t)j * rb->n_a], rb->n_a);
    poly.home_kind[j] = (rdeg == 0 && tdeg == 0) ? 0 : ((rdeg == 0 && tdeg == 1) ? 1 : 2);
    const double d0 = poly.D[j][0], c1 = rb->n_a > 1 ? poly.C[j][1] : 0.0;
    poly.helix_scale[j] = std::sqrt(1 + d0 * d0 * c1 * c1);
  }

  auto bail = [&](const char *what) { std::string m = what; tr_destroy(c); return fail(nullptr, TR_ERR_HIP, m); };
  if (hipMalloc((void **)&c->d_poly, sizeof(PolyK)) != hipSuccess) return bail("hipMalloc(poly)");
  if (hipMemcpy(c->d_poly, &poly, sizeof(PolyK), hipMemcpyHostToDevice) != hipSuccess) return bail("hipMemcpy(poly)");
  if (hipMalloc((void **)&c->d_tgrid, c->t.size() * sizeof(double)) != hipSuccess ||
      hipMalloc((void **)&c->d_hl, hl.size() * sizeof(double)) != hipSuccess) return bail("hipMalloc(tgrid)");
  if (hipMemcpy(c->d_tgrid, c->t.data(), c->t.size() * sizeof(double), hipMemcpyHostToDevice) != hipSuccess ||
      hipMemcpy(c->d_hl, hl.data(), hl.size() * sizeof(double), hipMemcpyHostToDevice) != hipSuccess) return bail("hipMemcpy(tgrid)");
  if (hipMalloc((void **)&c->d_tab, tab.size() * sizeof(double)) != hipSuccess) return bail("hipMalloc(tab)");
  if (hipMemcpy(c->d_tab, tab.data(), tab.size() * sizeof(double), hipMemcpyHostToDevice) != hipSuccess) return bail("hipMemcpy(tab)");
  if (hipMalloc((void **)&c->d_steps, std::max<size_t>(1, c->steps.size()) * sizeof(StepK)) != hipSuccess) return bail("hipMalloc(steps)");
  if (!c->steps.empty() &&
      hipMemcpy(c->d_steps, c->steps.data(), c->steps.size() * sizeof(StepK), hipMemcpyHostToDevice) != hipSuccess) return bail("hipMemcpy(steps)");
  *out = c;
  return TR_OK;
}

void tr_destroy(tr_ctx *c) {
  if (!c) return;
// ... 25 lines not shown
    if (sm.h_ctr) (void)hipHostFree(sm.h_ctr);
  }
  if (c->profile.d_table) (void)hipFree(c->profile.d_table);
  if (c->d_item_src) (void)hipFree(c->d_item_src);
  if (c->d_item_edge) (void)hipFree(c->d_item_edge);
  for (void *q : c->knn.p) if (q) (void)hipFree(q);
  if (c->vstore.ids) (void)hipFree(c->vstore.ids);
  if (c->vstore.masks) (void)hipFree(c->vstore.masks);
  if (c->edge.q_hctl) (void)hipHostFree(c->edge.q_hctl);
  if (c->edge.q_hargs) (void)hipHostFree(c->edge.q_hargs);
  if (c->h_stage) (void)hipHostFree(c->h_stage);
  for (auto &ln : c->lane) {
    tr_ctx::RetractOrder &ro = ln.ro;
    void *lp[] = {ln.counters, ln.fb_list, ln.fb_count, ro.keys[0], ro.keys[1], ro.vals[0], ro.vals[1], ro.kbegin, ro.handoff};
    for (void *q : lp) if (q) (void)hipFree(q);
    if (ln.stream) (void)hipStreamDestroy(ln.stream);
    if (ln.hc) (void)hipHostFree(ln.hc);
    trk::merge_free(ro.ms);
  }
  ik_release(c);
  shoot_release(c);
  ikl_release(c);
  c->ledge.pool.release(); c->ledge.out.release(); c->ledge.once.release();
  delete c;
}

int tr_state_size(const tr_ctx *c) { return c ? c->K.state_size : -1; }
int tr_set_loaded_retraction(tr_ctx *c, int on) {
  if (!c) return TR_ERR_INVALID_ARG;
  std::lock_guard<std::recursive_mutex> lock_(c->mu);
  c->loaded_retraction = on != 0;
  return TR_OK;
}
int tr_num_points(const tr_ctx *c) { return c ? c->K.n_points : -1; }
int tr_device(const tr_ctx *c) { return c ? c->device : -1; }

int tr_home_lengths(const tr_ctx *c, double *L_i) {
  if (!c || !L_i) return TR_ERR_INVALID_ARG;
  for (int j = 0; j < c->K.n_tendons; j++) L_i[j] = c->K.home_Li[j];
  return TR_OK;
}

int tr_set_checker(tr_ctx *c, int32_t checker) {
  if (!c) return TR_ERR_INVALID_ARG;
  std::lock_guard<std::recursive_mutex> lock_(c->mu);
  if (checker != TR_CHECKER_BACKBONE && checker != TR_CHECKER_SPHERES) return fail(c, TR_ERR_INVALID_ARG, "unknown checker");
  if (checker == TR_CHECKER_BACKBONE && c->has_grid && c->K.dL > std::max({c->G.dx, c->G.dy, c->G.dz}))
    return fail(c, TR_ERR_INVALID_ARG, "robot.specs.dL is larger than expected by VoxelBackboneValidityChecker");
  c->checker = checker;
  return TR_OK;
}

int tr_set_debug(tr_ctx *c, uint32_t bits) { if (!c) return TR_ERR_INVALID_ARG; c->debug = bits; return TR_OK; }
int tr_edge_schedule_last(const tr_ctx *c, uint32_t stats[4]) {
  if (!c || !stats) return TR_ERR_INVALID_ARG;
  for (int q = 0; q < 4; q++) stats[q] = c->edge_queue_last[q];
  return TR_OK;
}

int tr_set_grid(tr_ctx *c, uint32_t N, const double lim[6], const uint64_t *blocks, const double inv_rot[9]) {
  if (!c || !lim || !blocks) return fail(c, TR_ERR_INVALID_ARG, "null argument");
  std::lock_guard<std::recursive_mutex> lock_(c->mu);
  if (N < 4 || N > 512 || (N & (N - 1)))
    return fail(c, TR_ERR_INVALID_ARG, "unsupported voxel dimension: " + std::to_string(N));
  if (!(lim[0] < lim[1]) || !(lim[2] < lim[3]) || !(lim[4] < lim[5]))
    return fail(c, TR_ERR_LENGTH, "limits must be positive in size");
  GridK g{};
  g.N = (int)N; g.Nb = (int)N / 4;
  g.xmin = lim[0]; g.xmax = lim[1]; g.ymin = lim[2]; g.ymax = lim[3]; g.zmin = lim[4]; g.zmax = lim[5];
  g.dx = (g.xmax - g.xmin) / N; g.dy = (g.ymax - g.ymin) / N; g.dz = (g.zmax - g.zmin) / N;
  g.inv_dx = 1 / g.dx; g.inv_dy = 1 / g.dy; g.inv_dz = 1 / g.dz;
  const double max_dim = std::max({g.dx, g.dy, g.dz});
  if (c->checker == TR_CHECKER_BACKBONE && c->K.dL > max_dim) {
    char buf[160];
    snprintf(buf, sizeof buf, "robot.specs.dL is larger than expected by VoxelBackboneValidityChecker (%g > %g)", c->K.dL, max_dim);
    return fail(c, TR_ERR_INVALID_ARG, buf);
  }
  static const double I9[9] = {1, 0, 0, 0, 1, 0, 0, 0, 1};
  const double *r = inv_rot ? inv_rot : I9;
  g.rot_is_identity = 1;
  for (int i = 0; i < 9; i++) { g.inv_rot[i] = r[i]; if (r[i] != I9[i]) g.rot_is_identity = 0; }
  HIP_TRY(c, hipSetDevice(c->device));
  HIP_TRY(c, hipDeviceSynchronize());
  const size_t nb = (size_t)g.Nb * g.Nb * g.Nb;
  if (c->n_blocks != nb) {
    if (c->d_grid) { (void)hipFree(c->d_grid); c->d_grid = nullptr; }
    if (c->d_near) { (void)hipFree(c->d_near); c->d_near = nullptr; }
    HIP_TRY(c, hipMalloc((void **)&c->d_grid, nb * sizeof(uint64_t)));
    HIP_TRY(c, hipMalloc((void **)&c->d_near, nb * sizeof(uint64_t)));
    c->n_blocks = (uint32_t)nb;
  }
  HIP_TRY(c, hipMemcpy(c->d_grid, blocks, nb * sizeof(uint64_t), hipMemcpyHostToDevice));
  hipLaunchKernelGGL(trk::dilate2_blocks, dim3((unsigned)nb), dim3(64), 0, nullptr, c->d_grid, c->d_near, g.Nb);
  HIP_TRY(c, hipGetLastError());
  HIP_TRY(c, hipDeviceSynchronize());
  c->G = g;
  c->has_grid = true;
  c->sph_near_valid = false;
  return TR_OK;
}

namespace {
int env_begin(tr_ctx *c) {
  if (!c->has_grid) return fail(c, TR_ERR_INVALID_ARG, "no obstacle grid set (tr_set_grid)");
  HIP_TRY(c, hipSetDevice(c->device));
  HIP_TRY(c, hipDeviceSynchronize());
// ... 964 lines not shown
```

interactive-rate-tendons_amd/csrc/tr_types.hpp:

```cpp
#pragma once
#include <stdint.h>

#define TRK_MAX_TENDONS 8
#define TRK_MAX_COEF    8

struct RobotK {
  double ks0, ks2;
  double kb0, kb2;
  double dkb;
  double iks0, iks2;
  double ikb0, ikb2;
  double residual_threshold;
  double radius;
  double L, dL;
  double min_len[TRK_MAX_TENDONS];
  double max_len[TRK_MAX_TENDONS];
  double home_Li[TRK_MAX_TENDONS];
  double helix_omega, helix_rho2;
  int32_t n_tendons, n_a, n_m;
  int32_t enable_rotation, enable_retraction;
  int32_t state_size;
  int32_t n_points;
  int32_t routing_form;
};
#define TRK_ROUTING_TABLE 0
#define TRK_ROUTING_HELIX 1

struct PolyK {
  double C[TRK_MAX_TENDONS][TRK_MAX_COEF];
  double D[TRK_MAX_TENDONS][TRK_MAX_COEF];
  double helix_scale[TRK_MAX_TENDONS];
  int32_t home_kind[TRK_MAX_TENDONS];
};

struct StepK {
  double h;
  int32_t obs;
  int32_t pad_;
};

struct GridK {
  double xmin, xmax, ymin, ymax, zmin, zmax;
  double dx, dy, dz;
  double inv_dx, inv_dy, inv_dz;
  double inv_rot[9];
  int32_t N, Nb;
  int32_t rot_is_identity;
  int32_t pad_;
};

#ifndef TRK_K1_TWO_WAVE_MAXN
#define TRK_K1_TWO_WAVE_MAXN 6
#endif

namespace trk {

struct FkOut {
  double *__restrict__ px, *__restrict__ py, *__restrict__ pz;
  double *__restrict__ R;
  double *__restrict__ L;
  double *__restrict__ Li;
  double *__restrict__ tips;
  uint8_t *__restrict__ converged;
  int32_t *__restrict__ n_points;
  double *__restrict__ home_Li;
};

}
```

interactive-rate-tendons_amd/csrc/verdict_kernel.hpp:

```cpp
#pragma once
#include "fk_kernel.hpp"
#define TRK_DEVICE_BODIES_ONLY
#include "sweep_kernel.hpp"
#include "sphere_kernel.hpp"

namespace trk {

struct VerdictHot {
  double box[6];
  double org[3], inv_d[3];
  const uint64_t *near_grid;
  int32_t Nb, rot_is_identity, P, CH;
  int32_t use_near;
  int32_t pad_;
};
static_assert(sizeof(VerdictHot) == 128, "one 128-byte block");

struct alignas(128) VerdictArgs {
  VerdictHot hot;
  int P, CH, NM, pad0_;
  uint32_t debug, pad1_;
  double box[6];
  GridK g;
  const uint64_t *grid, *near_grid;
  uint64_t *valid_bits;
  uint8_t *flags;
  int32_t *fb_list;
  uint32_t *fb_count;
  uint32_t *sig;
  int64_t sig_stride;
  const float *field;
  float r_lo, r_hi;
  double radius;
  const int32_t *perm;
  int32_t *np_out;
  const int32_t *wave_k_begin;
  double home_Li[TRK_MAX_TENDONS], min_len[TRK_MAX_TENDONS], max_len[TRK_MAX_TENDONS];

  __host__ void finish_hot() {
    for (int q = 0; q < 6; q++) hot.box[q] = box[q];
    hot.org[0] = g.xmin; hot.org[1] = g.ymin; hot.org[2] = g.zmin;
    hot.inv_d[0] = g.inv_dx; hot.inv_d[1] = g.inv_dy; hot.inv_d[2] = g.inv_dz;
    hot.use_near = (near_grid != nullptr && !(debug & 4u)) ? 1 : 0;
    hot.near_grid = hot.use_near ? near_grid : grid;
    hot.Nb = g.Nb; hot.rot_is_identity = g.rot_is_identity; hot.P = P; hot.CH = CH;
  }
};

extern __shared__ double vlds[];
#ifndef TRK_SIG_VQ
#define TRK_SIG_VQ 88
#endif
template <bool SIG>
struct VLay {
  static constexpr int VQ = SIG ? TRK_SIG_VQ : 128;
  static constexpr int QE = 3 * 64;
  static constexpr int W0 = 2 * (QE + 6 * VQ);
  static constexpr int QOWNER = W0, OWNER_WORDS = SIG ? (VQ + 3) / 4 : VQ;
  static constexpr int CELL = QOWNER + OWNER_WORDS, INPREV = CELL + 3 * 64, HIT = INPREV + 64, DIST = HIT + 64, DELTA = DIST + 64, MS = DELTA + 64;
  static constexpr int NEARW = DELTA;
  __device__ static __forceinline__ int wrap(int i) {
    if constexpr ((VQ & (VQ - 1)) == 0) return i & (VQ - 1); else return i >= VQ ? i - VQ : i;
  }
  __device__ static __forceinline__ void set_owner(int slot, int lane) {
    if constexpr (SIG) ((uint8_t *)vlds)[4 * QOWNER + slot] = (uint8_t)lane; else ((uint32_t *)vlds)[QOWNER + slot] = (uint32_t)lane;
  }
  __device__ static __forceinline__ int owner(int slot) {
    if constexpr (SIG) return (int)((const uint8_t *)vlds)[4 * QOWNER + slot]; else return (int)((const uint32_t *)vlds)[QOWNER + slot];
  }
};
__host__ __device__ inline size_t verdict_lds_bytes(int NM, bool with_sig = false) {
  return (size_t)(with_sig ? VLay<true>::MS : VLay<false>::MS) * 4 + (size_t)4 * NM * 64 * sizeof(float) + (with_sig ? (size_t)SIG_LDS_WORDS * 4 : 0);
}

#define VL_D(i) (((double *)vlds)[(i)])
#define VL_U(i) (((uint32_t *)vlds)[(i)])
#define VL_I(i) (((int32_t *)vlds)[(i)])
#define VL_F(i) (((float *)vlds)[(i)])
#define VL_BARRIER() asm volatile("" ::: "memory")

template <bool SPH, bool SIG = false>
struct PointSweep {
  using Lay = VLay<SIG>;
  static constexpr int VQ = Lay::VQ;
  static constexpr int kLiInLdsFrom = (SIG && TRK_SIG_VQ > 88) ? (1 << 30) : 4;
  const VerdictArgs *va;
  float dn_prev;
  uint32_t sph_state;
  int qhead, qcount;
  int P, CH, NM, Kl, ms_next, ms_k;
  SigStage sigst;
  int sig_row_of, sig_first_row;
  int sig_row0, sig_cnt;
  bool active;

  __device__ __forceinline__ int sig_own_row() const { const int l = (int)threadIdx.x; return l < sig_cnt ? sig_row0 + l : -1; }
  __device__ __forceinline__ void sig_rows_of_launch(int64_t n) {
    const int64_t r0 = (int64_t)blockIdx.x * 64, left = n - r0;
    sig_row0 = (int)r0; sig_cnt = left >= 64 ? 64 : (left > 0 ? (int)left : 0);
  }
  __device__ __forceinline__ void sig_put(const VerdictArgs &a, int row, bool on, uint32_t value, int row_of, int first_row) {
    const int base = Lay::MS + 4 * NM * 64;
    sigst.put([base](int i) -> uint32_t & { return VL_U(base + i); }, a.sig, a.sig_stride, row_of, first_row, row, on, value);
  }
  template <bool RETRACT>
  __device__ __forceinline__ void sig_finish() {
    if constexpr (SIG) {
      const VerdictArgs &a = args();
      const int base = Lay::MS + 4 * NM * 64;
      sigst.flush([base](int i) -> uint32_t & { return VL_U(base + i); }, a.sig, a.sig_stride, RETRACT ? sig_row_of : sig_own_row(),
                  RETRACT ? sig_first_row : 0);
    }
  }

  __device__ __forceinline__ void begin(bool on) { active = on; }

  __device__ __forceinline__ const VerdictArgs &args() const {
    int zero = 0;
    asm volatile("" : "+s"(zero));
    return va[zero];
  }

  __device__ __forceinline__ void flush() {
#pragma clang fp contract(off)
    const VerdictArgs &a = args();
    const int lane = threadIdx.x;
    __syncthreads();
    const int cnt = qcount < 64 ? qcount : 64;
    if constexpr (SPH) {
      const GridK &g = a.g;
      const double radius = a.radius;
      for (int e = 0; e < cnt; e++) {
        const int slot = Lay::wrap(qhead + e);
        const double sx = VL_D(Lay::QE + 0 * VQ + slot), sy = VL_D(Lay::QE + 1 * VQ + slot), sz = VL_D(Lay::QE + 2 * VQ + slot);
        const int owner = Lay::owner(slot);
        bool found = false;
        {
          const double cx = fmin(fmax(sx, g.xmin), g.xmax), cy = fmin(fmax(sy, g.ymin), g.ymax), cz = fmin(fmax(sz, g.zmin), g.zmax);
          if (cx == sx && cy == sy && cz == sz) {
            const int N = g.N;
            int ix = (int)((cx - g.xmin) / g.dx), iy = (int)((cy - g.ymin) / g.dy), iz = (int)((cz - g.zmin) / g.dz);
            ix = ix < 0 ? 0 : (ix > N - 1 ? N - 1 : ix); iy = iy < 0 ? 0 : (iy > N - 1 ? N - 1 : iy); iz = iz < 0 ? 0 : (iz > N - 1 ? N - 1 : iz);
            found = ((a.grid[((size_t)(ix >> 2) * g.Nb + (iy >> 2)) * g.Nb + (iz >> 2)] >> (((ix & 3) << 4) | ((iy & 3) << 2) | (iz & 3))) & 1ull) != 0;
          }
        }
        if (!found) found = sphere_scan_wave(sx, sy, sz, radius, g, a.grid, lane);
        if (found && lane == 0) atomicOr(&((uint32_t *)vlds)[Lay::HIT + owner], 1u);
      }
    } else
    if (lane < cnt) {
      const int slot = Lay::wrap(qhead + lane);
      const V3 pa = {VL_D(Lay::QE + 0 * VQ + slot), VL_D(Lay::QE + 1 * VQ + slot), VL_D(Lay::QE + 2 * VQ + slot)};
      const V3 pb = {VL_D(Lay::QE + 3 * VQ + slot), VL_D(Lay::QE + 4 * VQ + slot), VL_D(Lay::QE + 5 * VQ + slot)};
      const int owner = Lay::owner(slot);
      V3 A, B;
      bool inside, bad = false, h = false;
      if (line_setup(pa, pb, a.g, A, B, inside, bad)) {
        GridCursor wc{a.grid, a.g.Nb, -1, 0ull};
        h = walk_cells(A, B, a.g, [&](int x, int y, int z) { return wc.occupied(x, y, z); });
      }
      if (h || bad) atomicOr(&((uint32_t *)vlds)[Lay::HIT + owner], (h ? 1u : 0u) | (bad ? 2u : 0u));
    }
    qhead = Lay::wrap(qhead + cnt);
    qcount -= cnt;
    __syncthreads();
  }

  __device__ __forceinline__ void request(const VerdictArgs &a, const V3 &q) {
#pragma clang fp contract(off)
    const GridK &g = a.g;
    V3 r = q;
    if (!g.rot_is_identity) {
      r.x = g.inv_rot[0] * q.x + g.inv_rot[1] * q.y + g.inv_rot[2] * q.z;
      r.y = g.inv_rot[3] * q.x + g.inv_rot[4] * q.y + g.inv_rot[5] * q.z;
      r.z = g.inv_rot[6] * q.x + g.inv_rot[7] * q.y + g.inv_rot[8] * q.z;
    }
    if (!(fabs(r.x) < 1e300) || !(fabs(r.y) < 1e300) || !(fabs(r.z) < 1e300)) return;
    const int N = g.N;
    const double cx = fmin(fmax(r.x, g.xmin), g.xmax), cy = fmin(fmax(r.y, g.ymin), g.ymax), cz = fmin(fmax(r.z, g.zmin), g.zmax);
    int ix = (int)((cx - g.xmin) / g.dx), iy = (int)((cy - g.ymin) / g.dy), iz = (int)((cz - g.zmin) / g.dz);
    ix = ix < 0 ? 0 : (ix > N - 1 ? N - 1 : ix); iy = iy < 0 ? 0 : (iy > N - 1 ? N - 1 : iy); iz = iz < 0 ? 0 : (iz > N - 1 ? N - 1 : iz);
    dn_prev = a.field[((size_t)ix * N + iy) * N + iz];
    sph_state = 1u | ((cx == r.x && cy == r.y && cz == r.z) ? 2u : 0u);
    const float ex = (float)(cx - (g.xmin + g.dx * ((double)ix + 0.5))), ey = (float)(cy - (g.ymin + g.dy * ((double)iy + 0.5))),
                ez = (float)(cz - (g.zmin + g.dz * ((double)iz + 0.5)));
    VL_F(Lay::DELTA + threadIdx.x) = sqrtf(ex * ex + ey * ey + ez * ez) * 1.000001f;
  }

  __device__ __forceinline__ void finish() {
#pragma clang fp contract(off)
    if constexpr (SPH) {
      VL_BARRIER();
      const VerdictArgs &a = args();
      const GridK &g = a.g;
      const int lane = threadIdx.x;
      bool need = false;
      V3 pr = {VL_D(lane), VL_D(64 + lane), VL_D(128 + lane)};
      if (active && !VL_U(Lay::HIT + lane) && (sph_state & 1u)) {
        if (!g.rot_is_identity) {
          const V3 pv = pr;
          pr.x = g.inv_rot[0] * pv.x + g.inv_rot[1] * pv.y + g.inv_rot[2] * pv.z;
          pr.y = g.inv_rot[3] * pv.x + g.inv_rot[4] * pv.y + g.inv_rot[5] * pv.z;
          pr.z = g.inv_rot[6] * pv.x + g.inv_rot[7] * pv.y + g.inv_rot[8] * pv.z;
        }
        const float dl = VL_F(Lay::DELTA + lane);
        if (dn_prev - dl > a.r_hi) {}
        else if ((sph_state & 2u) && dn_prev + dl < a.r_lo) VL_U(Lay::HIT + lane) = 1u;
        else need = true;
      }
      sph_state = 0;
      const unsigned long long wm = __ballot(need);
      if (wm) {
        if (qcount + __popcll(wm) > VQ) flush();
        if (need) {
          const int slot = Lay::wrap(qhead + qcount + __popcll(wm & (((unsigned long long)1 << lane) - 1)));
          VL_D(Lay::QE + 0 * VQ + slot) = pr.x; VL_D(Lay::QE + 1 * VQ + slot) = pr.y; VL_D(Lay::QE + 2 * VQ + slot) = pr.z;
          Lay::set_owner(slot, lane);
        }
        qcount += __popcll(wm);
      }
      VL_BARRIER();
    } else {
      asm volatile("s_waitcnt vmcnt(0)" ::: "memory");
    }
  }

  __device__ __forceinline__ void point_cell(const VerdictArgs &a, const V3 &q, V3 &qr, bool &in_q, int (&c)[3], double (&t)[3]) const {
#pragma clang fp contract(off)
    const VerdictHot &h = a.hot;
    qr = q;
    if (!h.rot_is_identity) {
      const GridK &g = a.g;
      qr.x = g.inv_rot[0] * q.x + g.inv_rot[1] * q.y + g.inv_rot[2] * q.z;
      qr.y = g.inv_rot[3] * q.x + g.inv_rot[4] * q.y + g.inv_rot[5] * q.z;
      qr.z = g.inv_rot[6] * q.x + g.inv_rot[7] * q.y + g.inv_rot[8] * q.z;
    }
    in_q = (qr.x > h.box[0]) & (qr.x < h.box[1]) & (qr.y > h.box[2]) & (qr.y < h.box[3]) & (qr.z > h.box[4]) & (qr.z < h.box[5]);
    t[0] = (qr.x - h.org[0]) * h.inv_d[0]; t[1] = (qr.y - h.org[1]) * h.inv_d[1]; t[2] = (qr.z - h.org[2]) * h.inv_d[2];
    c[0] = (int)t[0]; c[1] = (int)t[1]; c[2] = (int)t[2];
  }

  __device__ __forceinline__ uint32_t signature_of(const VerdictArgs &a, bool in_q, const int (&c)[3], const double (&t)[3],
                                                   double x, double y, double z) const {
#pragma clang fp contract(off)
    const double fx = t[0] - (double)c[0], fy = t[1] - (double)c[1], fz = t[2] - (double)c[2];
    const double lo = 1e-9, hi = 1.0 - 1e-9;
    const bool plain = in_q & (fx > lo) & (fx < hi) & (fy > lo) & (fy < hi) & (fz > lo) & (fz < hi);
    uint32_t sg = ((uint32_t)c[0] & 1023u) | (((uint32_t)c[1] & 1023u) << 10) | (((uint32_t)c[2] & 1023u) << 20);
    if (!plain) sg = cell_signature(x, y, z, a.g);
    return sg;
  }

  __device__ __forceinline__ bool voxel_test(const VerdictHot &h, bool first, bool in_q, const int (&c)[3]) {
    const int lane = threadIdx.x;
    const int cqx = c[0], cqy = c[1], cqz = c[2];
    const bool use_near = h.use_near != 0;
    const uint32_t was_in = VL_U(Lay::INPREV + lane);
    const int cpx = VL_I(Lay::CELL + lane), cpy = VL_I(Lay::CELL + 64 + lane), cpz = VL_I(Lay::CELL + 128 + lane);
    const uint32_t ex = (uint32_t)(cqx - cpx + 1), ey = (uint32_t)(cqy - cpy + 1), ez = (uint32_t)(cqz - cpz + 1);
    const uint32_t emax = ex > ey ? (ex > ez ? ex : ez) : (ey > ez ? ey : ez);
    const uint32_t bit = (uint32_t)(((cpx & 1) << 4) | ((cpy & 3) << 2) | (cpz & 3));
    asm volatile("s_waitcnt vmcnt(0)" ::: "memory");
    uint32_t near_bit = (VL_U(Lay::NEARW + lane) >> bit) & 1u;
    const bool start_free = use_near & (near_bit == 0u);
    const bool need = !first & !((was_in != 0u) & in_q & (emax <= 2u) & start_free);
    VL_I(Lay::CELL + lane) = cqx; VL_I(Lay::CELL + 64 + lane) = cqy; VL_I(Lay::CELL + 128 + lane) = cqz;
    VL_U(Lay::INPREV + lane) = in_q ? 1u : 0u;
    {
      const uint32_t nb = (uint32_t)h.Nb;
      uint32_t w = (((uint32_t)cqx >> 2) * nb + ((uint32_t)cqy >> 2)) * nb + ((uint32_t)cqz >> 2);
      w = in_q ? 2u * w + (((uint32_t)cqx >> 1) & 1u) : 0u;
      asm volatile("" : "+v"(w) : "v"(near_bit));
      typedef __attribute__((address_space(3))) uint32_t *lds_u32_ptr;
      __builtin_amdgcn_global_load_lds((const __attribute__((address_space(1))) uint32_t *)h.near_grid + w,
                                       (lds_u32_ptr)((uint32_t *)vlds + Lay::NEARW), 4, 0, 0);
    }
    return need;
  }

  __device__ __forceinline__ V3 to_voxel_frame(const VerdictArgs &a, const V3 &p) const {
#pragma clang fp contract(off)
    if (a.hot.rot_is_identity) return p;
    const GridK &g = a.g;
    return V3{g.inv_rot[0] * p.x + g.inv_rot[1] * p.y + g.inv_rot[2] * p.z, g.inv_rot[3] * p.x + g.inv_rot[4] * p.y + g.inv_rot[5] * p.z,
              g.inv_rot[6] * p.x + g.inv_rot[7] * p.y + g.inv_rot[8] * p.z};
  }

  __device__ __forceinline__ void operator()(int j, double x, double y, double z) {
#pragma clang fp contract(off)
    VL_BARRIER();
    const VerdictArgs &a = args();
    const GridK &g = a.g;
    const int lane = threadIdx.x;
    const V3 q = {x, y, z};
    V3 pv = q;
    float d = 0.0f;
    if (j > 0) { pv = V3{VL_D(lane), VL_D(64 + lane), VL_D(128 + lane)}; d = VL_F(Lay::DIST + lane); }
    {
      const float dx = (float)(q.x - pv.x), dy = (float)(q.y - pv.y), dz = (float)(q.z - pv.z);
      d += __builtin_amdgcn_sqrtf(dx * dx + dy * dy + dz * dz);
      VL_F(Lay::DIST + lane) = d;
    }
    if (j == ms_next) {
      const int CH_ = a.hot.CH, P_ = a.hot.P;
      const int o = Lay::MS + ms_k * 64 + lane, pl = a.NM * 64;
      VL_F(o) = (float)q.x; VL_F(o + pl) = (float)q.y; VL_F(o + 2 * pl) = (float)q.z; VL_F(o + 3 * pl) = d;
      ms_next = (ms_next + CH_ < P_ - 1) ? ms_next + CH_ : P_ - 1;
      ms_k++;
    }
    VL_D(lane) = q.x; VL_D(64 + lane) = q.y; VL_D(128 + lane) = q.z;
    bool need = false;
    V3 pr = pv, qr = q;
    bool in_q = false;
    int cq[3] = {0, 0, 0};
    if constexpr (!SPH) {
      double tq[3];
      point_cell(a, q, qr, in_q, cq, tq);
      if constexpr (SIG) sig_put(a, j, true, signature_of(a, in_q, cq, tq, x, y, z), sig_own_row(), 0);
    } else {
      if constexpr (SIG) sig_put(a, j, true, cell_signature(x, y, z, g), sig_own_row(), 0);
    }
    if constexpr (SPH) {
      if (active && !VL_U(Lay::HIT + lane)) {
        if (sph_state & 1u) {
          if (!g.rot_is_identity) {
            pr.x = g.inv_rot[0] * pv.x + g.inv_rot[1] * pv.y + g.inv_rot[2] * pv.z;
            pr.y = g.inv_rot[3] * pv.x + g.inv_rot[4] * pv.y + g.inv_rot[5] * pv.z;
            pr.z = g.inv_rot[6] * pv.x + g.inv_rot[7] * pv.y + g.inv_rot[8] * pv.z;
          }
          const float dl = VL_F(Lay::DELTA + lane);
          if (dn_prev - dl > a.r_hi) {}
          else if ((sph_state & 2u) && dn_prev + dl < a.r_lo) VL_U(Lay::HIT + lane) = 1u;
          else need = true;
        }
        sph_state = 0;
        if (!VL_U(Lay::HIT + lane)) request(a, q);
      }
    } else
    if (active && !VL_U(Lay::HIT + lane)) need = voxel_test(a.hot, j == 0, in_q, cq);
    const unsigned long long wm = __ballot(need);
    if (wm) {
      if (need) {
        if constexpr (!SPH) pr = to_voxel_frame(a, pv);
        const int slot = Lay::wrap(qhead + qcount + __popcll(wm & (((unsigned long long)1 << lane) - 1)));
        VL_D(Lay::QE + 0 * VQ + slot) = pr.x; VL_D(Lay::QE + 1 * VQ + slot) = pr.y; VL_D(Lay::QE + 2 * VQ + slot) = pr.z;
        if constexpr (!SPH) { VL_D(Lay::QE + 3 * VQ + slot) = qr.x; VL_D(Lay::QE + 4 * VQ + slot) = qr.y; VL_D(Lay::QE + 5 * VQ + slot) = qr.z; }
        Lay::set_owner(slot, lane);
      }
      qcount += __popcll(wm);
      if (qcount >= VQ - 64) flush();
    }
    VL_BARRIER();
  }

  __device__ __forceinline__ void tip_point(int row, bool on, bool first, double x, double y, double z, bool wave_row = true) {
#pragma clang fp contract(off)
    VL_BARRIER();
    const VerdictArgs &a = args();
    const GridK &g = a.g;
    const int lane = threadIdx.x;
    const V3 q = {x, y, z};
    V3 pv = q;
    bool need = false;
    V3 pr = pv, qr = q;
    bool in_q = false;
    int cq[3] = {0, 0, 0};
    double tq[3] = {0.0, 0.0, 0.0};
    if constexpr (!SPH) point_cell(a, q, qr, in_q, cq, tq);
    if constexpr (SIG) {
      uint32_t sg = 0u;
      if constexpr (!SPH) sg = on ? signature_of(a, in_q, cq, tq, x, y, z) : 0u;
      else sg = on ? cell_signature(x, y, z, g) : 0u;
      if (!wave_row) {
        if (on && sig_row_of >= 0) a.sig[(int64_t)sig_row_of * a.sig_stride + row] = sg;
        if (first) sig_first_row = row + 2;
      } else sig_put(a, row, on, sg, sig_row_of, sig_first_row);
    }
    if (on) {
      float d = 0.0f;
      if (!first) { pv = V3{VL_D(lane), VL_D(64 + lane), VL_D(128 + lane)}; d = VL_F(Lay::DIST + lane); }
      pr = pv;
      {
        const float dx = (float)(q.x - pv.x), dy = (float)(q.y - pv.y), dz = (float)(q.z - pv.z);
        d += __builtin_amdgcn_sqrtf(dx * dx + dy * dy + dz * dz);
        VL_F(Lay::DIST + lane) = d;
      }
      {
        const int back = P - 1 - row;
        const int k = (int)(((float)back + 0.5f) * (1.0f / (float)CH));
        const bool ms_row = (back - k * CH) == 0;
        if (first || ms_row) {
          const int slot = (first && !ms_row) ? k + 1 : k;
          const int o = Lay::MS + slot * 64 + lane, pl = NM * 64;
          VL_F(o) = (float)q.x; VL_F(o + pl) = (float)q.y; VL_F(o + 2 * pl) = (float)q.z; VL_F(o + 3 * pl) = -d;
        }
      }
      VL_D(lane) = q.x; VL_D(64 + lane) = q.y; VL_D(128 + lane) = q.z;
      if constexpr (SPH) {
        if (active && !VL_U(Lay::HIT + lane)) {
          if (sph_state & 1u) {
            if (!g.rot_is_identity) {
              pr.x = g.inv_rot[0] * pv.x + g.inv_rot[1] * pv.y + g.inv_rot[2] * pv.z;
              pr.y = g.inv_rot[3] * pv.x + g.inv_rot[4] * pv.y + g.inv_rot[5] * pv.z;
              pr.z = g.inv_rot[6] * pv.x + g.inv_rot[7] * pv.y + g.inv_rot[8] * pv.z;
            }
            const float dl = VL_F(Lay::DELTA + lane);
            if (dn_prev - dl > a.r_hi) {}
            else if ((sph_state & 2u) && dn_prev + dl < a.r_lo) VL_U(Lay::HIT + lane) = 1u;
            else need = true;
          }
          sph_state = 0;
          if (!VL_U(Lay::HIT + lane)) request(a, q);
        }
      } else
      if (active && !VL_U(Lay::HIT + lane)) need = voxel_test(a.hot, first, in_q, cq);
    }
    const unsigned long long wm = __ballot(need);
    if (wm) {
      if (need) {
        if constexpr (!SPH) pr = to_voxel_frame(a, pv);
        const int slot = Lay::wrap(qhead + qcount + __popcll(wm & (((unsigned long long)1 << lane) - 1)));
        VL_D(Lay::QE + 0 * VQ + slot) = pr.x; VL_D(Lay::QE + 1 * VQ + slot) = pr.y; VL_D(Lay::QE + 2 * VQ + slot) = pr.z;
        if constexpr (!SPH) { VL_D(Lay::QE + 3 * VQ + slot) = qr.x; VL_D(Lay::QE + 4 * VQ + slot) = qr.y; VL_D(Lay::QE + 5 * VQ + slot) = qr.z; }
        Lay::set_owner(slot, lane);
      }
      qcount += __popcll(wm);
      if (qcount >= VQ - 64) flush();
    }
    VL_BARRIER();
  }
};

struct LaneVerdict { bool valid, pending; uint32_t fl; };
template <int N, bool SPH, bool SIG>
__device__ __forceinline__ LaneVerdict verdict_decide(const VerdictArgs &a, const FkLane<N> &fl_, bool live) {
  using Lay = VLay<SIG>;
  const int lane = threadIdx.x;
  const int P = a.P;
  const int Kl = (P - 1 + a.CH - 1) / a.CH;
  const bool conv_ok = live && fl_.converged;
  bool len_ok = false;
  if (conv_ok) {
    bool ok = true;
#pragma unroll
    for (int j = 0; j < N; j++) {
      const double dl = a.home_Li[j] - fl_.Li[j];
      if (dl < a.min_len[j] || a.max_len[j] < dl) ok = false;
    }
    len_ok = ok;
  }
  bool alive = conv_ok && len_ok;
  const uint32_t hf = VL_U(Lay::HIT + lane);
  const bool hit = (hf & 1u) != 0;
  bool bad = (hf & 2u) != 0;
  if (alive && !(VL_F(Lay::DIST + lane) < 1e30f)) { alive = false; bad = true; }
  bool need_exact = alive && P > 2;
  if (!(a.debug & 2u) && __any(need_exact)) {
    const float *mx = (const float *)vlds + Lay::MS + lane, *my = mx + (size_t)a.NM * 64, *mz = my + (size_t)a.NM * 64, *ma = mz + (size_t)a.NM * 64;
    need_exact = milestones_unresolved(mx, my, mz, ma, a.NM, Kl, need_exact, (float)a.radius);
  }

  uint32_t fl = 0;
  if (conv_ok) fl |= 1u;
  if (conv_ok && len_ok) fl |= 2u;
  bool valid = conv_ok && len_ok;
  if (valid && bad) { fl |= 16u; valid = false; }
  const bool pending = valid && need_exact && (a.flags != nullptr || !hit);
  if (valid && !pending) {
    if (!need_exact) { fl |= 4u; if (!hit) fl |= 8u; else valid = false; }
    else valid = false;
  }
  if (pending) valid = false;
  if (SPH && pending && !hit) fl |= 8u;
  return LaneVerdict{valid, pending, fl};
}

#ifndef TRK_VERDICT_TWO_WAVE_MAXN
#define TRK_VERDICT_TWO_WAVE_MAXN 4
#endif
template <int N, bool ROT, bool SPH, bool SIG = false, class Form = TableRouting>
__global__ __launch_bounds__(64, (N <= TRK_VERDICT_TWO_WAVE_MAXN ? 2 : 1)) void fk_verdict(
    const double *__restrict__ states, int64_t n, RobotK K, const double *__restrict__ tab, const StepK *__restrict__ steps,
    int nsteps, double *__restrict__ tips, const VerdictArgs *__restrict__ va) {
  using Lay = VLay<SIG>;
  const int lane = threadIdx.x;
  PointSweep<SPH, SIG> ps;
  ps.va = va;
  ps.dn_prev = 0.0f; ps.sph_state = 0u;
  ps.qhead = 0; ps.qcount = 0; ps.active = false;
  ps.P = va->P; ps.CH = va->CH; ps.NM = va->NM; ps.Kl = (ps.P - 1 + ps.CH - 1) / ps.CH; ps.ms_next = 0; ps.ms_k = 0;
  VL_U(Lay::HIT + lane) = 0u; VL_U(Lay::INPREV + lane) = 0u; VL_F(Lay::DIST + lane) = 0.0f;
  {
    const int64_t i0 = (int64_t)blockIdx.x * 64 + lane;
    ps.sigst.init(); ps.sig_row_of = -1; ps.sig_first_row = 0; ps.sig_rows_of_launch(n);
  }
  __syncthreads();

  FkLane<N> fl_;
  FkOut out{nullptr, nullptr, nullptr, nullptr, nullptr, nullptr, nullptr, nullptr, nullptr, nullptr};
  fk_uniform_body<N, ROT, false, false, Form>(states, n, 0, K, tab, steps, nsteps, out, ps, nullptr, &fl_);

  ps.template sig_finish<false>();
  ps.finish();
  while (ps.qcount > 0) ps.flush();
  __syncthreads();
  if (tips) {
    VL_D(lane) = fl_.tip[0]; VL_D(64 + lane) = fl_.tip[1]; VL_D(128 + lane) = fl_.tip[2];
    __syncthreads();
    const int64_t e0 = (int64_t)blockIdx.x * 192, etot = 3 * n;
#pragma unroll
    for (int q = 0; q < 3; q++) {
      const int e = q * 64 + lane;
      if (e0 + e < etot) tips[e0 + e] = VL_D((e % 3) * 64 + e / 3);
    }
    __syncthreads();
  }
  const VerdictArgs a = *va;
  const int64_t i = (int64_t)blockIdx.x * 64 + lane;
  const bool live = i < n;
  const LaneVerdict lv = verdict_decide<N, SPH, SIG>(a, fl_, live);
  const bool valid = lv.valid, pending = lv.pending;
  const uint32_t fl = lv.fl;
  const uint64_t bits = __ballot(valid && live);
  if (lane == 0 && live) a.valid_bits[i >> 6] = bits;
  if (a.flags && live) a.flags[i] = (uint8_t)fl;
  const unsigned long long pm = __ballot(pending);
  if (pm) {
    uint32_t base = 0;
    if (lane == 0) base = atomicAdd(a.fb_count, (uint32_t)__popcll(pm));
    base = __shfl(base, 0, 64);
    if (pending) a.fb_list[base + __popcll(pm & (((unsigned long long)1 << lane) - 1))] = (int32_t)i;
  }
}

#ifdef TRK_WITH_RETRACT_VERDICT
template <int N, bool ROT, bool SPH, bool SIG = false>
__global__ __launch_bounds__(64, (N <= TRK_VR_TWO_WAVE_MAXN ? 2 : 1)) void fk_verdict_retract(
    const double *__restrict__ states, int64_t n, RobotK K, const PolyK *__restrict__ pk, const double *__restrict__ tab,
    const StepK *__restrict__ steps, int nsteps, int k_first, const double *__restrict__ tgrid, const double *__restrict__ hl,
    double *__restrict__ tips, const VerdictArgs *__restrict__ va, RetractHandoff ho) {
  using Lay = VLay<SIG>;
  const int lane = threadIdx.x;
  PointSweep<SPH, SIG> ps;
  ps.va = va;
  ps.dn_prev = 0.0f; ps.sph_state = 0u;
  ps.qhead = 0; ps.qcount = 0; ps.active = false;
  ps.P = va->P; ps.CH = va->CH; ps.NM = va->NM; ps.Kl = 0; ps.ms_next = 0; ps.ms_k = 0;
  const int32_t *__restrict__ perm = va->perm;
  {
    const int64_t i0 = (int64_t)blockIdx.x * 64 + lane;
    ps.sigst.init(); ps.sig_row_of = i0 < n ? (perm ? perm[i0] : (int)i0) : -1; ps.sig_first_row = 0; ps.sig_row0 = 0; ps.sig_cnt = 0;
  }
  VL_U(Lay::HIT + lane) = 0u; VL_U(Lay::INPREV + lane) = 0u; VL_F(Lay::DIST + lane) = 0.0f;
  __syncthreads();

  FkLaneR<N> fl_;
  FkOut out{nullptr, nullptr, nullptr, nullptr, nullptr, nullptr, tips, nullptr, nullptr, nullptr};
  const int32_t *__restrict__ wkb = va->wave_k_begin;
  fk_retract_body<N, ROT, false, PointSweep<SPH, SIG> &, 2>(states, n, 0, K, pk, tab, steps, nsteps, k_first, tgrid, hl, out, ps, perm, &fl_,
                                                            wkb ? wkb[blockIdx.x] : 0, &ho);

  ps.template sig_finish<true>();
  ps.finish();
  while (ps.qcount > 0) ps.flush();
  __syncthreads();
  const VerdictArgs a = *va;
  const int64_t i = (int64_t)blockIdx.x * 64 + lane;
  const bool live = i < n;
  const int64_t c = (perm && live) ? (int64_t)perm[i] : i;
  const int np = fl_.np;
  const int Kl = (np - 1 + a.CH - 1) / a.CH;
  const bool conv_ok = live && fl_.converged;
  bool len_ok = false;
  if (conv_ok) {
    bool ok = true;
#pragma unroll
    for (int j = 0; j < N; j++) {
      const double dl = fl_.home_Li[j] - fl_.Li[j];
      if (dl < a.min_len[j] || a.max_len[j] < dl) ok = false;
    }
    len_ok = ok;
  }
  bool alive = conv_ok && len_ok;
  const uint32_t hf = VL_U(Lay::HIT + lane);
  const bool hit = (hf & 1u) != 0;
  bool bad = (hf & 2u) != 0;
  if (alive && !(VL_F(Lay::DIST + lane) < 1e30f)) { alive = false; bad = true; }
  bool need_exact = alive && np > 2;
  if (!(a.debug & 2u) && __any(need_exact)) {
    const float *mx = (const float *)vlds + Lay::MS + lane, *my = mx + (size_t)a.NM * 64, *mz = my + (size_t)a.NM * 64, *ma = mz + (size_t)a.NM * 64;
    need_exact = milestones_unresolved(mx, my, mz, ma, a.NM, Kl, need_exact, (float)a.radius);
  }

  uint32_t fl = 0;
  if (conv_ok) fl |= 1u;
  if (conv_ok && len_ok) fl |= 2u;
  bool valid = conv_ok && len_ok;
  if (valid && bad) { fl |= 16u; valid = false; }
  const bool pending = valid && need_exact && (a.flags != nullptr || !hit);
  if (valid && !pending) {
    if (!need_exact) { fl |= 4u; if (!hit) fl |= 8u; else valid = false; }
    else valid = false;
  }
  if (pending) valid = false;
  if (SPH && pending && !hit) fl |= 8u;
  if (perm) {
// ... 37 lines not shown
```

interactive-rate-tendons_amd/engine.py:

```python
import contextlib
import ctypes as C

import numpy as np

from . import _lib as L


def _dp(a):
    return a.ctypes.data_as(C.POINTER(C.c_double))


def _f64(a):
    return np.ascontiguousarray(np.asarray(a, dtype=np.float64))


def _torch():
    import torch
    return torch


def unpack_bits(words, n):
    w = np.ascontiguousarray(words, dtype=np.uint64)
    return np.unpackbits(w.view(np.uint8), bitorder="little")[:n].astype(bool)

# ... 111 lines not shown
            pass

    def home_lengths(self):
        out = np.zeros(self.n_tendons)
        L.check(self._ctx, self.lib.tr_home_lengths(self._ctx, _dp(out)))
        return out

    def set_grid(self, N, limits, blocks, inv_rot=None):
        lim = _f64(limits).reshape(6)
        blk = np.ascontiguousarray(blocks, dtype=np.uint64).reshape(-1)
        if blk.size != (N // 4) ** 3:
            raise L.InvalidArgument("voxel dimension mismatch (%d blocks for N=%d)" % (blk.size, N))
        rot = None if inv_rot is None else _f64(inv_rot).reshape(9)
        L.check(self._ctx, self.lib.tr_set_grid(self._ctx, int(N), _dp(lim),
                                                blk.ctypes.data_as(C.POINTER(C.c_uint64)),
                                                _dp(rot) if rot is not None else None))
        self.has_grid = True
        self._grid_nb = (int(N) // 4) ** 3

    def grid_add_spheres(self, spheres):
        sp = _f64(spheres).reshape(-1, 4)
        L.check(self._ctx, self.lib.tr_grid_add_spheres(self._ctx, _dp(sp), sp.shape[0]))

    def grid_add_capsules(self, capsules):
        cp = _f64(capsules).reshape(-1, 7)
        L.check(self._ctx, self.lib.tr_grid_add_capsules(self._ctx, _dp(cp), cp.shape[0]))

    def grid_remove_interior(self, keep_diagonal=True):
        L.check(self._ctx, self.lib.tr_grid_remove_interior(self._ctx, int(bool(keep_diagonal))))

    def grid_dilate(self, num=1, use_diagonal=False):
        L.check(self._ctx, self.lib.tr_grid_dilate(self._ctx, int(num), int(bool(use_diagonal))))

    def grid_dilate_sphere(self, r):
        L.check(self._ctx, self.lib.tr_grid_dilate_sphere(self._ctx, float(r)))

    def get_grid(self):
        blk = np.empty(self._grid_nb, dtype=np.uint64)
        L.check(self._ctx, self.lib.tr_get_grid(self._ctx, blk.ctypes.data_as(C.POINTER(C.c_uint64))))
        return blk

    def set_checker(self, spheres):
        L.check(self._ctx, self.lib.tr_set_checker(self._ctx, L.TR_CHECKER_SPHERES if spheres else L.TR_CHECKER_BACKBONE))

    def reserve(self, n):
        L.check(self._ctx, self.lib.tr_reserve(self._ctx, int(n)))

    def reserve_edges(self, n_edges):
        L.check(self._ctx, self.lib.tr_reserve_edges(self._ctx, int(n_edges)))

    def set_debug(self, bits):
        L.check(self._ctx, self.lib.tr_set_debug(self._ctx, int(bits)))

    def edge_schedule_last(self):
        st = (C.c_uint32 * 4)()
        L.check(self._ctx, self.lib.tr_edge_schedule_last(self._ctx, st))
        return dict(samples=int(st[0]), rounds=int(st[1]), exact_sweep=int(st[2]), flags=int(st[3]))

    def _states(self, states):
        st = _f64(states)
        if st.ndim == 1:
            st = st.reshape(1, -1)
        if st.ndim != 2 or st.shape[1] != self.state_size:
            raise L.InvalidArgument("State is not the right size")
        return st

    def fk_batch(self, states, want_R=False):
        st = self._states(states)
        n, P, N = st.shape[0], self.num_points, self.n_tendons
        p = np.empty((n, P, 3))
        R = np.empty((n, P, 9)) if want_R else None
        Lb, Li = np.empty(n), np.empty((n, N))
        conv = np.empty(n, dtype=np.uint8)
        npts = np.empty(n, dtype=np.int32)
        L.check(self._ctx, self.lib.tr_fk_batch(self._ctx, _dp(st), n, _dp(p), _dp(R) if want_R else None,
                                                _dp(Lb), _dp(Li), conv.ctypes.data_as(C.POINTER(C.c_uint8)),
                                                npts.ctypes.data_as(C.POINTER(C.c_int32))))
        return dict(p=p, R=R, L=Lb, L_i=Li, converged=conv.astype(bool), n_points=npts)

    def fk_tips(self, states):
        st = self._states(states)
        n = st.shape[0]
        tips = np.empty((n, 3))
        conv = np.empty(n, dtype=np.uint8)
        L.check(self._ctx, self.lib.tr_fk_tips(self._ctx, _dp(st), n, _dp(tips), conv.ctypes.data_as(C.POINTER(C.c_uint8))))
        return tips, conv.astype(bool)

    def fk_tips_dev(self, d_states, n, d_tips, d_conv=None, stream=None):
        torch = _torch()
        ps = self._check_dev(d_states, torch.float64, n * self.state_size, "d_states")
        pt = self._check_dev(d_tips, torch.float64, 3 * n, "d_tips")
        pc = self._check_dev(d_conv, torch.uint8, n, "d_conv") if d_conv is not None else None
        L.check(self._ctx, self.lib.tr_fk_tips_dev(self._ctx, ps, int(n), pt, pc, self._stream_ptr(stream)))

    def tip_jacobian(self, states, delta=1e-6, want_tips=False):
        st = self._states(states)
        n, S = st.shape
        J = np.empty((n, 3, S))
        tips = np.empty((n, 3)) if want_tips else None
        L.check(self._ctx, self.lib.tr_tip_jacobian(self._ctx, _dp(st), n, float(delta), _dp(tips) if want_tips else None, _dp(J)))
        return (J, tips) if want_tips else J

    def tip_jacobian_dev(self, d_states, n, d_J, delta=1e-6, d_tips=None, stream=None):
        torch = _torch()
        S = self.state_size
        ps = self._check_dev(d_states, torch.float64, n * S, "d_states")
# ... 964 lines not shown
```

profiles/count_isa.py:

```python
#!/usr/bin/env python3
import collections
import json
import os
import re
import subprocess
import sys
import tempfile

ROOT = os.path.dirname(os.path.dirname(os.path.abspath(__file__)))
CSRC = os.path.join(ROOT, "interactive-rate-tendons_amd", "csrc")
OUT = os.path.join(ROOT, "profiles", "isa_counts.json")
FLAGS = ["--offload-arch=gfx950", "-O3", "-std=c++17", "-ffp-contract=off"]

FLOPS = {"v_fma_f64": 2, "v_fmac_f64": 2, "v_mul_f64": 1, "v_add_f64": 1, "v_rcp_f64": 1, "v_rsq_f64": 1, "v_sqrt_f64": 1,
         "v_div_fmas_f64": 2, "v_div_fixup_f64": 1, "v_div_scale_f64": 1, "v_pk_fma_f64": 4, "v_pk_mul_f64": 2,
         "v_pk_add_f64": 2}

_RK4_ONLY = r'''
#include <hip/hip_runtime.h>
#include "tr_types.hpp"
#include "fk_kernel.hpp"
namespace trk {
// the RK4 step as fk_verdict and fk_sweep_fused hold it (no rotation, no R output, no backbone-length quadrature), without
// any per-point hook: the reference count of useful flops per step
template <int N> __global__ __launch_bounds__(64, 2) void rk4_step_only(const double *states, int64_t n, int64_t ld, RobotK K,
                                                                         const double *tab, const StepK *steps, int nsteps, FkOut out) {
  fk_uniform_body<N, false, false, false>(states, n, ld, K, tab, steps, nsteps, out);
}
}
template __global__ void trk::rk4_step_only<%d>(const double*, int64_t, int64_t, RobotK, const double*, const StepK*, int, trk::FkOut);
'''

_RK4_ONLY_HELIX = r'''
#include <hip/hip_runtime.h>
#include "tr_types.hpp"
#include "fk_kernel.hpp"
namespace trk {
template <int N> __global__ __launch_bounds__(64, 2) void rk4_step_only_helix(const double *states, int64_t n, int64_t ld, RobotK K,
                                                                               const double *tab, const StepK *steps, int nsteps, FkOut out) {
  fk_uniform_body<N, false, false, false, UniformHelix>(states, n, ld, K, tab, steps, nsteps, out);
}
}
template __global__ void trk::rk4_step_only_helix<%d>(const double*, int64_t, int64_t, RobotK, const double*, const StepK*, int, trk::FkOut);
'''

KERNELS = {
    "rk4_step<3>": _RK4_ONLY % 3,
    "rk4_step<4>": _RK4_ONLY % 4,
    "fk_verdict<3,false>": r'''
#include <hip/hip_runtime.h>
#include "tr_types.hpp"
#include "verdict_kernel.hpp"
template __global__ void trk::fk_verdict<3, false, false>(const double*, int64_t, RobotK, const double*, const StepK*, int, double*, const trk::VerdictArgs*);
''',
    "fk_verdict<4,false>": r'''
#include <hip/hip_runtime.h>
#include "tr_types.hpp"
#include "verdict_kernel.hpp"
template __global__ void trk::fk_verdict<4, false, false>(const double*, int64_t, RobotK, const double*, const StepK*, int, double*, const trk::VerdictArgs*);
''',
    "fk_sweep_fused<3,false>": r'''
#include <hip/hip_runtime.h>
#include "tr_types.hpp"
#include "fused_kernel.hpp"
template __global__ void trk::fk_sweep_fused<3, false>(const double*, int64_t, int64_t, RobotK, const double*, const StepK*, int,
                                                       trk::FkOut, const trk::FusedSweepArgs*);
''',
    "fk_sweep_fused<4,false>": r'''
#include <hip/hip_runtime.h>
#include "tr_types.hpp"
#include "fused_kernel.hpp"
template __global__ void trk::fk_sweep_fused<4, false>(const double*, int64_t, int64_t, RobotK, const double*, const StepK*, int,
                                                       trk::FkOut, const trk::FusedSweepArgs*);
''',
    "fk_rk4_batch_uniform<3,false,false>": r'''
#include <hip/hip_runtime.h>
#include "tr_types.hpp"
#include "fk_kernel.hpp"
template __global__ void trk::fk_rk4_batch_uniform<3, false, false>(const double*, int64_t, int64_t, RobotK,
                                                                     const double*, const StepK*, int, trk::FkOut);
''',
    "fk_rk4_batch_uniform<4,false,false>": r'''
#include <hip/hip_runtime.h>
#include "tr_types.hpp"
#include "fk_kernel.hpp"
template __global__ void trk::fk_rk4_batch_uniform<4, false, false>(const double*, int64_t, int64_t, RobotK,
                                                                     const double*, const StepK*, int, trk::FkOut);
''',
    "rk4_step_helix<3>": _RK4_ONLY_HELIX % 3,
    "rk4_step_helix<4>": _RK4_ONLY_HELIX % 4,
    "fk_verdict_helix<3,false>": r'''
#include <hip/hip_runtime.h>
#include "tr_types.hpp"
#include "verdict_kernel.hpp"
template __global__ void trk::fk_verdict<3, false, false, false, trk::UniformHelix>(const double*, int64_t, RobotK, const double*, const StepK*, int, double*, const trk::VerdictArgs*);
''',
    "fk_sweep_fused_helix<3,false>": r'''
#include <hip/hip_runtime.h>
#include "tr_types.hpp"
#include "fused_kernel.hpp"
template __global__ void trk::fk_sweep_fused<3, false, trk::UniformHelix>(const double*, int64_t, int64_t, RobotK, const double*, const StepK*, int,
                                                                          trk::FkOut, const trk::FusedSweepArgs*);
''',
}

_BLOCK = re.compile(r"^(\.LBB\d+_\d+):\s*(?:;\s*(.*))?$")
_FALL = re.compile(r"^; (%bb\.\d+):\s*(?:;\s*(.*))?$")
_HDR = re.compile(r"Header=(BB\d+_\d+)")
_INSN = re.compile(r"^\s+([vs]_[a-z0-9_]+)")


def count_asm(asm):
    blocks = []
    cur, hist, nv = None, collections.Counter(), 0
    for line in asm.splitlines():
        m = _BLOCK.match(line) or _FALL.match(line)
        if m:
            blocks.append((cur, hist, nv))
            hist, nv = collections.Counter(), 0
            note = m.group(2) or ""
            if "Loop Header" in note and "This" in note:
                cur = m.group(1)[2:] if m.group(1).startswith(".L") else None
            else:
                h = _HDR.search(note)
                cur = h.group(1) if h else None
            continue
        m = _INSN.match(line)
        if not m:
            continue
        op = m.group(1)
        for suffix in ("_e32", "_e64", "_dpp", "_sdwa"):
            if op.endswith(suffix):
                op = op[: -len(suffix)]
        if op.startswith("v_"):
            nv += 1
            if op.endswith("_f64"):
                hist[op] += 1
    blocks.append((cur, hist, nv))
    loops = collections.defaultdict(collections.Counter)
    valu, rare = collections.Counter(), collections.Counter()
    for hdr, h, n in blocks:
        if hdr is None:
            continue
        if any(op.startswith("v_div_") for op in h):
            rare[hdr] += 1
            continue
        loops[hdr].update(h)
        valu[hdr] += n
# ... 47 lines not shown
```

profiles/kbench.hip:

```cpp
#include <hip/hip_runtime.h>
#include <algorithm>
#include <cmath>
#include <cstdio>
#include <cstdlib>
#include <vector>
#include "tr_types.hpp"
#include "fk_kernel.hpp"
#ifdef KB_VERDICT
#include "verdict_kernel.hpp"
#ifdef KB_SIG
constexpr bool kSig = true;
#else
constexpr bool kSig = false;
#endif
#endif

#ifndef KB_N
#define KB_N 3
#endif
#ifdef KB_HELIX
static_assert(KB_N == 3, "-DKB_HELIX: only the KB_N == 3 robot is a uniform helix");
using KbForm = trk::UniformHelix;
#else
using KbForm = trk::TableRouting;
#endif
#ifndef KB_LOG2
#define KB_LOG2 20
#endif
#ifndef KB_REPS
#define KB_REPS 7
#endif
#ifndef KB_WAVES
#define KB_WAVES 2
#endif

namespace trk {
template <int N> __global__ __launch_bounds__(64, KB_WAVES) void rk4_only(const double *__restrict__ states, int64_t n, RobotK K,
                                                                           const double *__restrict__ tab, const StepK *__restrict__ steps,
                                                                           int nsteps, double *__restrict__ tips) {
  FkOut out{nullptr, nullptr, nullptr, nullptr, nullptr, nullptr, tips, nullptr, nullptr, nullptr};
  fk_uniform_body<N, false, false, false, KbForm>(states, n, 0, K, tab, steps, nsteps, out);
}
}

#define CK(x) do { hipError_t e_ = (x); if (e_ != hipSuccess) { std::fprintf(stderr, "%s: %s\n", #x, hipGetErrorString(e_)); return 1; } } while (0)

static void routing_at(int N, const double C[][3], const double D[][3], double t, double *out) {
  for (int j = 0; j < N; j++) {
    const double th = C[j][0] + C[j][1] * t + C[j][2] * t * t, th1 = C[j][1] + 2 * C[j][2] * t, th2 = 2 * C[j][2];
    const double rho = D[j][0] + D[j][1] * t + D[j][2] * t * t, rho1 = D[j][1] + 2 * D[j][2] * t, rho2 = 2 * D[j][2];
    const double sa = std::sin(th), ca = std::cos(th);
    double *o = out + 6 * j;
    o[0] = rho * sa; o[1] = rho * ca;
    o[2] = rho1 * sa + rho * (ca * th1);
    o[3] = rho1 * ca + rho * (-sa * th1);
    o[4] = rho2 * sa + 2 * rho1 * (ca * th1) - rho * (sa * th1 * th1) + rho * (ca * th2);
    o[5] = rho2 * ca + 2 * rho1 * (-sa * th1) - rho * (ca * th1 * th1) + rho * (-sa * th2);
  }
}

int main() {
  constexpr int N = KB_N;
  const double L = 0.2, dL = L / 128, ro = 0.01, ri = 0.0, E = 2.1e6, nu = 0.3;
  double C[8][3] = {}, D[8][3] = {};
  if (N == 3) for (int k = 0; k < 3; k++) { C[k][0] = 2 * M_PI * k / 3; C[k][1] = 5.0; D[k][0] = 0.01; }
  else {
    const double c1[4] = {3.0, -2.0, 4.0, -5.0}, c2[4] = {10.0, 15.0, -12.0, 8.0}, d1[4] = {-0.01, 0.005, 0.0, -0.005};
    for (int k = 0; k < N; k++) { C[k][0] = M_PI * k / 2; C[k][1] = c1[k % 4]; C[k][2] = c2[k % 4]; D[k][0] = 0.01; D[k][1] = d1[k % 4]; }
  }
  RobotK K{};
  {
    const double ro2 = ro * ro, ri2 = ri * ri, I = 0.25 * M_PI * (ro2 * ro2 - ri2 * ri2), Ar = M_PI * (ro2 - ri2), J = 2 * I, G = E / (2 * (1 + nu));
    K.kb0 = E * I; K.kb2 = J * G; K.dkb = K.kb2 - K.kb0; K.ikb0 = 1 / K.kb0; K.ikb2 = 1 / K.kb2; K.ks0 = G * Ar; K.ks2 = E * Ar; K.iks0 = 1 / K.ks0; K.iks2 = 1 / K.ks2;
  }
#ifdef KB_HELIX
  K.routing_form = TRK_ROUTING_HELIX; K.helix_omega = C[0][1]; K.helix_rho2 = D[0][0] * D[0][0];
#endif
  K.residual_threshold = 5e-6; K.radius = 0.015; K.L = L; K.dL = dL; K.n_tendons = N; K.n_a = 3; K.n_m = 3; K.state_size = N; K.n_points = 129;
  std::vector<StepK> steps;
  std::vector<double> tab((1 + 3 * 128) * N * 6);
  routing_at(N, C, D, 0.0, tab.data());
  for (int k = 0; k < 128; k++) {
    const double tk = k * dL;
    steps.push_back(StepK{dL, k + 1, 0});
    for (int q = 0; q < 3; q++) routing_at(N, C, D, tk + 0.5 * q * dL, &tab[(size_t)(1 + 3 * k + q) * N * 6]);
  }
#ifdef KB_COUNT
  const int64_t n = KB_COUNT;
#else
  const int64_t n = (int64_t)1 << KB_LOG2;
#endif
  std::vector<double> st((size_t)n * N);
  unsigned long long lcg = 88172645463325252ull;
  const double tmax = N == 3 ? 10.0 : 20.0;
  for (auto &x : st) { lcg = lcg * 6364136223846793005ull + 1442695040888963407ull; x = tmax * (double)(lcg >> 11) * (1.0 / 9007199254740992.0); }
  double *d_st, *d_tab, *d_tips; StepK *d_steps;
  CK(hipMalloc(&d_st, st.size() * 8)); CK(hipMalloc(&d_tab, tab.size() * 8)); CK(hipMalloc(&d_tips, (size_t)n * 24)); CK(hipMalloc(&d_steps, steps.size() * sizeof(StepK)));
  CK(hipMemcpy(d_st, st.data(), st.size() * 8, hipMemcpyHostToDevice)); CK(hipMemcpy(d_tab, tab.data(), tab.size() * 8, hipMemcpyHostToDevice));
  CK(hipMemcpy(d_steps, steps.data(), steps.size() * sizeof(StepK), hipMemcpyHostToDevice));
  hipEvent_t a, b; CK(hipEventCreate(&a)); CK(hipEventCreate(&b));
#ifdef KB_VERDICT
  trk::VerdictArgs va{};
  va.P = 129; va.CH = (int)std::lround(2.0 * K.radius / dL); va.NM = (128 + va.CH - 1) / va.CH + 1;
  GridK &g = va.g;
  g.xmin = g.ymin = g.zmin = -0.25; g.xmax = g.ymax = g.zmax = 0.25; g.N = 256; g.Nb = 64; g.rot_is_identity = 1;
  g.dx = g.dy = g.dz = 0.5 / 256; g.inv_dx = g.inv_dy = g.inv_dz = 1 / g.dx;
  for (int q = 0; q < 9; q++) g.inv_rot[q] = (q % 4 == 0) ? 1.0 : 0.0;
  for (int q = 0; q < 3; q++) { va.box[2 * q] = -0.25 + 1e-6 * 0.5; va.box[2 * q + 1] = 0.25 - 1e-6 * 0.5; }
  uint64_t *d_grid, *d_bits; int32_t *d_fb; uint32_t *d_fbc; trk::VerdictArgs *d_va;
  CK(hipMalloc(&d_grid, (size_t)64 * 64 * 64 * 8 * 2)); CK(hipMemset(d_grid, 0, (size_t)64 * 64 * 64 * 8 * 2));
  CK(hipMalloc(&d_bits, (size_t)((n + 63) / 64) * 8)); CK(hipMalloc(&d_fb, (size_t)n * 4)); CK(hipMalloc(&d_fbc, 4)); CK(hipMemset(d_fbc, 0, 4));
  va.grid = d_grid; va.near_grid = d_grid + 64 * 64 * 64; va.valid_bits = d_bits; va.fb_list = d_fb; va.fb_count = d_fbc;
  va.radius = K.radius;
  uint32_t *d_sig = nullptr;
  if (kSig) { va.sig_stride = (129 + 15) / 16 * 16; CK(hipMalloc(&d_sig, (size_t)n * va.sig_stride * 4)); va.sig = d_sig; }
  for (int j = 0; j < N; j++) { va.min_len[j] = K.min_len[j] = -1.0; va.max_len[j] = K.max_len[j] = 1.0; va.home_Li[j] = K.home_Li[j] = L; }
  va.finish_hot();
  CK(hipMalloc(&d_va, sizeof(va))); CK(hipMemcpy(d_va, &va, sizeof(va), hipMemcpyHostToDevice));
  const size_t lds = trk::verdict_lds_bytes(va.NM, kSig);
#endif
  std::vector<float> ms;
  for (int r = 0; r < KB_REPS + 2; r++) {
    CK(hipEventRecord(a));
#ifdef KB_VERDICT
    hipLaunchKernelGGL((trk::fk_verdict<N, false, false, kSig, KbForm>), dim3((unsigned)((n + 63) / 64)), dim3(64), lds, nullptr, d_st, n, K, d_tab, d_steps, 128, d_tips, d_va);
#else
    hipLaunchKernelGGL((trk::rk4_only<N>), dim3((unsigned)((n + 63) / 64)), dim3(64), 0, nullptr, d_st, n, K, d_tab, d_steps, 128, d_tips);
#endif
    CK(hipEventRecord(b)); CK(hipEventSynchronize(b));
    float t; CK(hipEventElapsedTime(&t, a, b));
    if (r >= 2) ms.push_back(t);
  }
  std::vector<double> tips((size_t)n * 3);
  CK(hipMemcpy(tips.data(), d_tips, tips.size() * 8, hipMemcpyDeviceToHost));
  double sum = 0, asum = 0; for (double v : tips) { sum += v; asum += std::fabs(v); }
  std::sort(ms.begin(), ms.end());
  hipFuncAttributes fa;
#ifdef KB_VERDICT
  CK(hipFuncGetAttributes(&fa, (const void *)trk::fk_verdict<N, false, false, kSig, KbForm>));
  {
    std::vector<uint64_t> bits((size_t)((n + 63) / 64));
    CK(hipMemcpy(bits.data(), d_bits, bits.size() * 8, hipMemcpyDeviceToHost));
    uint32_t fbc = 0; CK(hipMemcpy(&fbc, d_fbc, 4, hipMemcpyDeviceToHost));
    long valid = 0; for (uint64_t w : bits) valid += __builtin_popcountll(w);
    std::printf("fk_verdict: valid %ld of %ld, fallback entries %u (summed over launches)\n", valid, (long)n, fbc);
  }
#else
  CK(hipFuncGetAttributes(&fa, (const void *)trk::rk4_only<N>));
#endif
#ifdef KB_HELIX
  std::printf("routing form: uniform helix   ");
#else
  std::printf("routing form: table   ");
#endif
  std::printf("N=%d n=%ld (2^%d unless KB_COUNT) waves/SIMD<=%d: best %.3f ms  median %.3f ms  -> %.4g FK/s   regs %d  scratch %zu B   tips sum %.17g abs %.17g\n", N, (long)n, KB_LOG2, KB_WAVES,
              ms.front(), ms[ms.size() / 2], (double)n / (ms.front() * 1e-3), fa.numRegs, (size_t)fa.localSizeBytes, sum, asum);
  return 0;
}
```

Baseline: 135.7 million.

## Add fast-hook verdict kernel variant with precomputed milestone slots and LDS-cached hot args

Adds a FAST template variant of the fused FK+voxel verdict kernel for identity rotation with the near grid, no spheres and no signatures, with N ≤ 4. The host now precomputes per-step milestone slots into the former padding of StepK, so the kernel no longer tracks milestone counters at run time. The hot verdict arguments are staged in LDS, with the previous-point area moved to make room. This aims to cut registers and scalar work in the per-point hook, at the cost of more template instantiations, a slightly changed LDS layout (SIG VQ drops from 88 to 85), and a new query API for which variant ran.

```diff
diff --git a/include/tendon_hip.h b/include/tendon_hip.h
--- a/include/tendon_hip.h
+++ b/include/tendon_hip.h
@@ -434,6 +434,7 @@
 int tr_set_debug(tr_ctx *ctx, uint32_t bits);
 
 int tr_edge_schedule_last(const tr_ctx *ctx, uint32_t stats[4]);
+int tr_verdict_hook_last(const tr_ctx *ctx, int32_t *variant);
 
 
 #ifdef __cplusplus
diff --git a/interactive-rate-tendons_amd/_lib.py b/interactive-rate-tendons_amd/_lib.py
--- a/interactive-rate-tendons_amd/_lib.py
+++ b/interactive-rate-tendons_amd/_lib.py
@@ -26,7 +26,7 @@
     "tr_check_cached", "tr_check_cached_dev", "tr_check_cached_subset_dev", "tr_state_layout", "tr_space_weights", "tr_kstar_k",
     "tr_roadmap_create", "tr_roadmap_destroy", "tr_roadmap_last_error", "tr_roadmap_set_caches", "tr_roadmap_set_caches_dev", "tr_roadmap_prepare", "tr_roadmap_clear_validity",
     "tr_roadmap_revalidate", "tr_roadmap_get_validity", "tr_roadmap_set_validity", "tr_roadmap_solve", "tr_roadmap_fetch_paths", "tr_roadmap_search_stats", "tr_roadmap_profile", "tr_roadmap_release_search_state", "tr_roadmap_reserve_search_state", "tr_roadmap_search_state_bytes", "tr_roadmap_search_sweeps", "tr_voxelize_batch", "tr_voxelize_edges", "tr_voxelize_edges_indexed", "tr_connect_edges_indexed", "tr_voxelize_fetch", "tr_voxelize_fetch_dev", "tr_voxelize_count", "tr_knn", "tr_knn_range", "tr_knn_table_edges", "tr_knn_edges", "tr_knn_edges_dev", "tr_knn_range_dev", "tr_knn_table_edges_dev", "tr_validate_edges_indexed_dev", "tr_signature_words", "tr_signature_packed_words", "tr_pack_signatures_dev", "tr_unpack_signatures_dev", "tr_validate_candidates_sig_dev", "tr_validate_edges_indexed_sig_dev", "tr_profile_begin", "tr_profile_read", "tr_profile_end",
-    "tr_set_debug", "tr_edge_schedule_last",
+    "tr_set_debug", "tr_edge_schedule_last", "tr_verdict_hook_last",
     "tr_candidate_states", "tr_candidate_states_dev", "tr_validate_candidates_dev", "tr_compact_rows_dev",
     "tr_sample_valid_vertices", "tr_sample_valid_vertices_dev", "tr_sample_valid_vertices_sig_dev",
     "tr_fk_tips", "tr_fk_tips_dev", "tr_tip_jacobian", "tr_tip_jacobian_dev", "tr_ik_batch", "tr_ik_batch_dev",
@@ -409,6 +409,7 @@
     L.tr_profile_end.argtypes = [vp]
     L.tr_set_debug.argtypes = [vp, C.c_uint32]
     L.tr_edge_schedule_last.argtypes = [vp, P(C.c_uint32)]
+    L.tr_verdict_hook_last.argtypes = [vp, P(C.c_int32)]
     _lib = L
     return L
 
diff --git a/interactive-rate-tendons_amd/csrc/edge_queue_kernel.hpp b/interactive-rate-tendons_amd/csrc/edge_queue_kernel.hpp
--- a/interactive-rate-tendons_amd/csrc/edge_queue_kernel.hpp
+++ b/interactive-rate-tendons_amd/csrc/edge_queue_kernel.hpp
@@ -153,13 +153,9 @@
     clk.lap(q.ctl, EQ_T_READY);
 
     PointSweep<false, true> ps;
-    ps.va = va;
-    ps.dn_prev = 0.0f; ps.sph_state = 0u;
-    ps.qhead = 0; ps.qcount = 0; ps.active = false;
-    ps.P = va->P; ps.CH = va->CH; ps.NM = va->NM; ps.Kl = (ps.P - 1 + ps.CH - 1) / ps.CH; ps.ms_next = 0; ps.ms_k = 0;
-    ps.sigst.init(); ps.sig_row_of = -1; ps.sig_first_row = 0; ps.sig_row0 = h; ps.sig_cnt = cnt;
     __syncthreads();
-    VL_U(VLay<true>::HIT + lane) = 0u; VL_U(VLay<true>::INPREV + lane) = 0u; VL_F(VLay<true>::DIST + lane) = 0.0f;
+    ps.init(va);
+    ps.sig_row0 = h; ps.sig_cnt = cnt;
     __syncthreads();
     const int S = K.state_size;
     const double *st_eff = q.states + ((int64_t)h - (int64_t)blockIdx.x * 64) * S;
diff --git a/interactive-rate-tendons_amd/csrc/fk_inst.hip b/interactive-rate-tendons_amd/csrc/fk_inst.hip
--- a/interactive-rate-tendons_amd/csrc/fk_inst.hip
+++ b/interactive-rate-tendons_amd/csrc/fk_inst.hip
@@ -120,20 +120,25 @@
   if (a.rotation) go_list<true>(a, sweep, lds, list, count); else go_list<false>(a, sweep, lds, list, count);
 }
 #elif TRK_INST_KIND == 3
-template <bool ROT, bool SPH, bool SIG, class Form>
+template <bool ROT, bool SPH, bool SIG, class Form, bool FAST = false>
 static void go(const FkLaunch &a, const VerdictArgs *va, size_t lds) {
   const unsigned grid = (unsigned)((a.n + 63) / 64);
-  hipLaunchKernelGGL((fk_verdict<TRK_INST_N, ROT, SPH, SIG, Form>), dim3(grid), dim3(64), lds, a.stream, a.d_states, a.n, a.K, a.d_tab, a.d_steps,
+  hipLaunchKernelGGL((fk_verdict<TRK_INST_N, ROT, SPH, SIG, Form, FAST>), dim3(grid), dim3(64), lds, a.stream, a.d_states, a.n, a.K, a.d_tab, a.d_steps,
                      a.n_steps, a.out.tips, va);
 }
-template <bool SPH, bool SIG>
+template <bool SPH, bool SIG, bool FAST = false>
 static void go_rot(const FkLaunch &a, const VerdictArgs *va, size_t lds) {
-  if (helix_form(a.K)) { if (a.rotation) go<true, SPH, SIG, HelixForm>(a, va, lds); else go<false, SPH, SIG, HelixForm>(a, va, lds); }
-  else                 { if (a.rotation) go<true, SPH, SIG, TableRouting>(a, va, lds); else go<false, SPH, SIG, TableRouting>(a, va, lds); }
+  if (helix_form(a.K)) { if (a.rotation) go<true, SPH, SIG, HelixForm, FAST>(a, va, lds); else go<false, SPH, SIG, HelixForm, FAST>(a, va, lds); }
+  else                 { if (a.rotation) go<true, SPH, SIG, TableRouting, FAST>(a, va, lds); else go<false, SPH, SIG, TableRouting, FAST>(a, va, lds); }
 }
-template <> void launch_fk_verdict<TRK_INST_N>(const FkLaunch &a, const VerdictArgs *va, size_t lds, bool spheres, bool with_sig) {
+constexpr bool kFastHookKernels = TRK_INST_N <= 4;
+template <> bool launch_fk_verdict<TRK_INST_N>(const FkLaunch &a, const VerdictArgs *va, size_t lds, bool spheres, bool with_sig, bool fast_hook) {
+  if constexpr (kFastHookKernels) {
+    if (fast_hook && !spheres && !with_sig) { go_rot<false, false, true>(a, va, lds); return true; }
+  }
   if (spheres) { if (with_sig) go_rot<true, true>(a, va, lds); else go_rot<true, false>(a, va, lds); }
   else         { if (with_sig) go_rot<false, true>(a, va, lds); else go_rot<false, false>(a, va, lds); }
+  return false;
 }
 #elif TRK_INST_KIND == 2
 template <bool ROT, class Form>
diff --git a/interactive-rate-tendons_amd/csrc/fk_kernel.hpp b/interactive-rate-tendons_amd/csrc/fk_kernel.hpp
--- a/interactive-rate-tendons_amd/csrc/fk_kernel.hpp
+++ b/interactive-rate-tendons_amd/csrc/fk_kernel.hpp
@@ -357,7 +357,7 @@
 
 struct NoPointHook {
   __device__ __forceinline__ void begin(bool) const {}
-  __device__ __forceinline__ void operator()(int, double, double, double) const {}
+  __device__ __forceinline__ void operator()(int, double, double, double, int = -1) const {}
   __device__ __forceinline__ void tip_point(int, bool, bool, double, double, double, bool = true) const {}
 };
 
@@ -408,11 +408,11 @@
 #pragma unroll
   for (int j = 0; j < N; j++) Li[j] = 0;
 
-  auto store_point = [&](int j) {
+  auto store_point = [&](int j, int ms) {
     const int64_t o = (int64_t)j * ld + i;
     double x = p[0], y = p[1], z = p[2];
     if (ROT) { const double x2 = __builtin_fma(rc, x, -(rs * y)), y2 = __builtin_fma(rs, x, rc * y); x = x2; y = y2; z = r22 * z; }
-    on_point(j, x, y, z);
+    on_point(j, x, y, z, ms);
     if (!live) return;
     if (out.px) { out.px[o] = x; out.py[o] = y; out.pz[o] = z; }
     if (WRITE_R) {
@@ -425,11 +425,11 @@
       }
     }
   };
-  store_point(0);
+  store_point(0, 0);
 
   for (int k = 0; k < nsteps; k++) {
     const double h = steps[k].h;
-    const int obs = steps[k].obs;
+    const int obs = steps[k].obs, ms = steps[k].ms;
     const double *__restrict__ rt = tab + (size_t)(1 + 3 * k) * (N * 6);
     const double hh = h * 0.5;
     const double b1 = h * (1.0 / 6.0), b2 = h * (1.0 / 3.0);
@@ -477,7 +477,7 @@
     for (int q = 0; q < 9; q++) R[q] = __builtin_fma(b1, aR[q], R[q]);
 #pragma unroll
     for (int q = 0; q < 3; q++) { v[q] = av[q]; u[q] = au[q]; }
-    if (obs >= 0) store_point(obs);
+    if (obs >= 0) store_point(obs, ms);
   }
 
   if constexpr (kLiLds) {
diff --git a/interactive-rate-tendons_amd/csrc/fk_launch.hpp b/interactive-rate-tendons_amd/csrc/fk_launch.hpp
--- a/interactive-rate-tendons_amd/csrc/fk_launch.hpp
+++ b/interactive-rate-tendons_amd/csrc/fk_launch.hpp
@@ -35,7 +35,7 @@
 template <int N> void launch_fk_sweep_fused(const FkLaunch &a, const FusedSweepArgs *sweep, size_t lds);
 template <int N> void launch_fk_sweep_fused_list(const FkLaunch &a, const FusedSweepArgs *sweep, size_t lds, const int32_t *list,
                                                  const uint32_t *count);
-template <int N> void launch_fk_verdict(const FkLaunch &a, const VerdictArgs *va, size_t lds, bool spheres, bool with_sig);
+template <int N> bool launch_fk_verdict(const FkLaunch &a, const VerdictArgs *va, size_t lds, bool spheres, bool with_sig, bool fast_hook);
 template <int N> void launch_fk_retract(const FkLaunch &a);
 template <int N> void launch_fk_verdict_retract(const FkLaunch &a, const VerdictArgs *va, size_t lds, bool spheres, bool with_sig);
 template <int N> void launch_fk_sweep_retract_list(const FkLaunch &a, const FusedSweepArgs *sweep, size_t lds, const int32_t *list,
@@ -58,7 +58,7 @@
   template <> void launch_shoot_start_retract<N>(const FkLaunch &, const double *, double *); \
   template <> void launch_fk_sweep_fused<N>(const FkLaunch &, const FusedSweepArgs *, size_t); \
   template <> void launch_fk_sweep_fused_list<N>(const FkLaunch &, const FusedSweepArgs *, size_t, const int32_t *, const uint32_t *); \
-  template <> void launch_fk_verdict<N>(const FkLaunch &, const VerdictArgs *, size_t, bool, bool); \
+  template <> bool launch_fk_verdict<N>(const FkLaunch &, const VerdictArgs *, size_t, bool, bool, bool); \
   template <> void launch_fk_verdict_retract<N>(const FkLaunch &, const VerdictArgs *, size_t, bool, bool); \
   template <> void launch_fk_sweep_retract_list<N>(const FkLaunch &, const FusedSweepArgs *, size_t, const int32_t *, const uint32_t *); \
   template <> void launch_fk_edge_queue<N>(const FkLaunch &, const VerdictArgs *, size_t, const EdgeQueueArgs *, const FusedSweepArgs *, unsigned); \
diff --git a/interactive-rate-tendons_amd/csrc/sweep_kernel.hpp b/interactive-rate-tendons_amd/csrc/sweep_kernel.hpp
--- a/interactive-rate-tendons_amd/csrc/sweep_kernel.hpp
+++ b/interactive-rate-tendons_amd/csrc/sweep_kernel.hpp
@@ -277,7 +277,7 @@
   __device__ __forceinline__ static uint32_t &word(int i) { extern __shared__ float lds[]; return ((uint32_t *)lds)[i]; }
   __device__ __forceinline__ int row_of() const { const int64_t i = (int64_t)blockIdx.x * 64 + threadIdx.x; return i < n ? (int)i : -1; }
   __device__ __forceinline__ void begin(bool) const {}
-  __device__ __forceinline__ void operator()(int j, double x, double y, double z) {
+  __device__ __forceinline__ void operator()(int j, double x, double y, double z, int = -1) {
     if (!any) return;
     int zero = 0;
     asm volatile("" : "+s"(zero));
diff --git a/interactive-rate-tendons_amd/csrc/tendon_hip.hip b/interactive-rate-tendons_amd/csrc/tendon_hip.hip
--- a/interactive-rate-tendons_amd/csrc/tendon_hip.hip
+++ b/interactive-rate-tendons_amd/csrc/tendon_hip.hip
@@ -149,6 +149,7 @@
   int64_t edge_slots_max = 1 << 24;
   int64_t edge_slots_now = 0;
   double ch_scale = 2.0;
+  int verdict_hook_last = -1;
   int64_t k1_round = 1 << 17;
   int fuse = 2;
   int64_t fb_cap = 1 << 17;
@@ -769,7 +770,7 @@
     ProfScope ps(ctx, 5, s);
     switch (ctx->K.n_tendons) {
 #define TRK_CASE(N) case N: if (ret) trk::launch_fk_verdict_retract<N>(vl, vr.d_slots + vslot, lds_v, spheres, sig != nullptr); \
-                            else trk::launch_fk_verdict<N>(vl, vr.d_slots + vslot, lds_v, spheres, sig != nullptr); break;
+                            else ctx->verdict_hook_last = trk::launch_fk_verdict<N>(vl, vr.d_slots + vslot, lds_v, spheres, sig != nullptr, a.fast_hook()) ? 1 : 0; break;
       TRK_CASE(1) TRK_CASE(2) TRK_CASE(3) TRK_CASE(4) TRK_CASE(5) TRK_CASE(6) TRK_CASE(7) TRK_CASE(8)
 #undef TRK_CASE
       default: return fail(ctx, TR_ERR_OUT_OF_RANGE, "n_tendons out of range");
@@ -1002,13 +1003,18 @@
     bool any = false;
     while (tn - cur > DBL_EPSILON) {
       const double h = std::min(rb->dL, tn - cur);
-      c->steps.push_back(StepK{h, -1, 0});
+      c->steps.push_back(StepK{h, -1, -1});
       step_t.push_back(cur);
       cur += h;
       any = true;
     }
-    if (!any) { c->steps.push_back(StepK{0.0, -1, 0}); step_t.push_back(cur); }
+    if (!any) { c->steps.push_back(StepK{0.0, -1, -1}); step_t.push_back(cur); }
     c->steps.back().obs = (int)j + 1;
+  }
+  {
+    int CH, NM; size_t lds;
+    sweep_geometry(c, CH, NM, lds);
+    fill_milestone_slots(c->steps, K.n_points, CH);
   }
   const size_t ent = (size_t)N * 6;
   std::vector<double> tab((1 + 3 * c->steps.size()) * ent);
@@ -1140,6 +1146,12 @@
 }
 
 int tr_set_debug(tr_ctx *c, uint32_t bits) { if (!c) return TR_ERR_INVALID_ARG; c->debug = bits; return TR_OK; }
+int tr_verdict_hook_last(const tr_ctx *c, int32_t *variant) {
+  if (!c || !variant) return TR_ERR_INVALID_ARG;
+  *variant = c->verdict_hook_last;
+  return TR_OK;
+}
+
 int tr_edge_schedule_last(const tr_ctx *c, uint32_t stats[4]) {
   if (!c || !stats) return TR_ERR_INVALID_ARG;
   for (int q = 0; q < 4; q++) stats[q] = c->edge_queue_last[q];
diff --git a/interactive-rate-tendons_amd/csrc/tr_types.hpp b/interactive-rate-tendons_amd/csrc/tr_types.hpp
--- a/interactive-rate-tendons_amd/csrc/tr_types.hpp
+++ b/interactive-rate-tendons_amd/csrc/tr_types.hpp
@@ -36,8 +36,17 @@
 struct StepK {
   double h;
   int32_t obs;
-  int32_t pad_;
+  int32_t ms;
 };
+static_assert(sizeof(StepK) == 16, "one 16-byte record per step: h, obs and ms arrive in one scalar load");
+
+inline int milestone_slot(int j, int P, int CH) {
+  if (j == P - 1) return (P - 1 + CH - 1) / CH;
+  return (j % CH) == 0 ? j / CH : -1;
+}
+template <class Steps> inline void fill_milestone_slots(Steps &steps, int P, int CH) {
+  for (auto &s : steps) s.ms = s.obs >= 0 ? milestone_slot(s.obs, P, CH) : -1;
+}
 
 struct GridK {
   double xmin, xmax, ymin, ymax, zmin, zmax;
diff --git a/interactive-rate-tendons_amd/csrc/verdict_kernel.hpp b/interactive-rate-tendons_amd/csrc/verdict_kernel.hpp
--- a/interactive-rate-tendons_amd/csrc/verdict_kernel.hpp
+++ b/interactive-rate-tendons_amd/csrc/verdict_kernel.hpp
@@ -12,9 +12,13 @@
   const uint64_t *near_grid;
   int32_t Nb, rot_is_identity, P, CH;
   int32_t use_near;
-  int32_t pad_;
+  int32_t ms_plane;
 };
 static_assert(sizeof(VerdictHot) == 128, "one 128-byte block");
+constexpr int kHotNearGridD = 12, kHotNbW = 26, kHotRotW = 27, kHotUseNearW = 30, kHotMsPlaneW = 31;
+static_assert(offsetof(VerdictHot, near_grid) == 8 * kHotNearGridD && offsetof(VerdictHot, Nb) == 4 * kHotNbW &&
+              offsetof(VerdictHot, rot_is_identity) == 4 * kHotRotW && offsetof(VerdictHot, use_near) == 4 * kHotUseNearW &&
+              offsetof(VerdictHot, ms_plane) == 4 * kHotMsPlaneW, "VerdictHot: field offsets as the LDS copy is read");
 
 struct alignas(128) VerdictArgs {
   VerdictHot hot;
@@ -43,18 +47,19 @@
     hot.inv_d[0] = g.inv_dx; hot.inv_d[1] = g.inv_dy; hot.inv_d[2] = g.inv_dz;
     hot.use_near = (near_grid != nullptr && !(debug & 4u)) ? 1 : 0;
     hot.near_grid = hot.use_near ? near_grid : grid;
-    hot.Nb = g.Nb; hot.rot_is_identity = g.rot_is_identity; hot.P = P; hot.CH = CH;
-  }
+    hot.Nb = g.Nb; hot.rot_is_identity = g.rot_is_identity; hot.P = P; hot.CH = CH; hot.ms_plane = 64 * NM;
+  }
+  __host__ bool fast_hook() const { return hot.rot_is_identity != 0 && hot.use_near != 0; }
 };
 
-extern __shared__ double vlds[];
+extern __shared__ __attribute__((aligned(16))) double vlds[];
 #ifndef TRK_SIG_VQ
-#define TRK_SIG_VQ 88
+#define TRK_SIG_VQ 85
 #endif
 template <bool SIG>
 struct VLay {
   static constexpr int VQ = SIG ? TRK_SIG_VQ : 128;
-  static constexpr int QE = 3 * 64;
+  static constexpr int HOT = 0, PREV = 16, QE = PREV + 3 * 64;
   static constexpr int W0 = 2 * (QE + 6 * VQ);
   static constexpr int QOWNER = W0, OWNER_WORDS = SIG ? (VQ + 3) / 4 : VQ;
   static constexpr int CELL = QOWNER + OWNER_WORDS, INPREV = CELL + 3 * 64, HIT = INPREV + 64, DIST = HIT + 64, DELTA = DIST + 64, MS = DELTA + 64;
@@ -79,16 +84,18 @@
 #define VL_F(i) (((float *)vlds)[(i)])
 #define VL_BARRIER() asm volatile("" ::: "memory")
 
-template <bool SPH, bool SIG = false>
+struct HotBox { double box[6], org[3], inv_d[3]; };
+template <bool SPH, bool SIG = false, bool FAST = false>
 struct PointSweep {
+  static_assert(!FAST || !SPH, "the sphere checker has the generic hook only");
   using Lay = VLay<SIG>;
   static constexpr int VQ = Lay::VQ;
-  static constexpr int kLiInLdsFrom = (SIG && TRK_SIG_VQ > 88) ? (1 << 30) : 4;
+  static constexpr int kLiInLdsFrom = (SIG && TRK_SIG_VQ > 85) ? (1 << 30) : 4;
   const VerdictArgs *va;
   float dn_prev;
   uint32_t sph_state;
   int qhead, qcount;
-  int P, CH, NM, Kl, ms_next, ms_k;
+  int P, CH, NM, Kl;
   SigStage sigst;
   int sig_row_of, sig_first_row;
   int sig_row0, sig_cnt;
@@ -113,7 +120,29 @@
     }
   }
 
-  __device__ __forceinline__ void begin(bool on) { active = on; }
+  __device__ __forceinline__ void begin(bool on) { active = on; if (!on) VL_U(Lay::HIT + (int)threadIdx.x) = 4u; }
+
+  __device__ __forceinline__ void init(const VerdictArgs *__restrict__ va_) {
+    const int lane = threadIdx.x;
+    va = va_;
+    dn_prev = 0.0f; sph_state = 0u;
+    qhead = 0; qcount = 0; active = false;
+    P = va_->P; CH = va_->CH; NM = va_->NM; Kl = (P - 1 + CH - 1) / CH;
+    if (lane < 16) VL_D(Lay::HOT + lane) = ((const double *)&va_->hot)[lane];
+    VL_U(Lay::HIT + lane) = 0u; VL_U(Lay::INPREV + lane) = 0u; VL_F(Lay::DIST + lane) = 0.0f;
+    sigst.init(); sig_row_of = -1; sig_first_row = 0; sig_row0 = 0; sig_cnt = 0;
+  }
+  __device__ __forceinline__ static HotBox hot_box() {
+    HotBox h;
+#pragma unroll
+    for (int q = 0; q < 6; q++) h.box[q] = VL_D(Lay::HOT + q);
+#pragma unroll
+    for (int q = 0; q < 3; q++) { h.org[q] = VL_D(Lay::HOT + 6 + q); h.inv_d[q] = VL_D(Lay::HOT + 9 + q); }
+    return h;
+  }
+  __device__ __forceinline__ static int hot_word(int w) { return VL_I(2 * Lay::HOT + w); }
+  __device__ __forceinline__ static bool rot_is_identity() { return FAST || __builtin_amdgcn_readfirstlane(hot_word(kHotRotW)) != 0; }
+  __device__ __forceinline__ static bool use_near() { return FAST || hot_word(kHotUseNearW) != 0; }
 
   __device__ __forceinline__ const VerdictArgs &args() const {
     int zero = 0;
@@ -195,7 +224,7 @@
       const GridK &g = a.g;
       const int lane = threadIdx.x;
       bool need = false;
-      V3 pr = {VL_D(lane), VL_D(64 + lane), VL_D(128 + lane)};
+      V3 pr = {VL_D(Lay::PREV + lane), VL_D(Lay::PREV + 64 + lane), VL_D(Lay::PREV + 128 + lane)};
       if (active && !VL_U(Lay::HIT + lane) && (sph_state & 1u)) {
         if (!g.rot_is_identity) {
           const V3 pv = pr;
@@ -225,12 +254,11 @@
     }
   }
 
-  __device__ __forceinline__ void point_cell(const VerdictArgs &a, const V3 &q, V3 &qr, bool &in_q, int (&c)[3], double (&t)[3]) const {
-#pragma clang fp contract(off)
-    const VerdictHot &h = a.hot;
+  __device__ __forceinline__ void point_cell(const HotBox &h, const V3 &q, V3 &qr, bool &in_q, int (&c)[3], double (&t)[3]) const {
+#pragma clang fp contract(off)
     qr = q;
-    if (!h.rot_is_identity) {
-      const GridK &g = a.g;
+    if (!rot_is_identity()) {
+      const GridK &g = args().g;
       qr.x = g.inv_rot[0] * q.x + g.inv_rot[1] * q.y + g.inv_rot[2] * q.z;
       qr.y = g.inv_rot[3] * q.x + g.inv_rot[4] * q.y + g.inv_rot[5] * q.z;
       qr.z = g.inv_rot[6] * q.x + g.inv_rot[7] * q.y + g.inv_rot[8] * q.z;
@@ -251,28 +279,42 @@
     return sg;
   }
 
-  __device__ __forceinline__ bool voxel_test(const VerdictHot &h, bool first, bool in_q, const int (&c)[3]) {
+  struct VoxelState { uint32_t was_in, nearw, nb; int cpx, cpy, cpz; const uint64_t *near_grid; };
+  __device__ __forceinline__ static void request_landed() { asm volatile("s_waitcnt vmcnt(0)" ::: "memory"); }
+  __device__ __forceinline__ static VoxelState voxel_state() {
+    const int lane = threadIdx.x;
+    VoxelState v;
+    v.was_in = VL_U(Lay::INPREV + lane);
+    v.cpx = VL_I(Lay::CELL + lane); v.cpy = VL_I(Lay::CELL + 64 + lane); v.cpz = VL_I(Lay::CELL + 128 + lane);
+    v.nearw = VL_U(Lay::NEARW + lane);
+    v.nb = (uint32_t)hot_word(kHotNbW);
+    v.near_grid = ((const uint64_t *const *)vlds)[Lay::HOT + kHotNearGridD];
+    return v;
+  }
+  __device__ __forceinline__ bool voxel_test(const VoxelState &vs, bool first, bool in_q, const int (&c)[3]) {
     const int lane = threadIdx.x;
     const int cqx = c[0], cqy = c[1], cqz = c[2];
-    const bool use_near = h.use_near != 0;
-    const uint32_t was_in = VL_U(Lay::INPREV + lane);
-    const int cpx = VL_I(Lay::CELL + lane), cpy = VL_I(Lay::CELL + 64 + lane), cpz = VL_I(Lay::CELL + 128 + lane);
+    const bool use_near = PointSweep::use_near();
+    const uint32_t was_in = vs.was_in;
+    const int cpx = vs.cpx, cpy = vs.cpy, cpz = vs.cpz;
     const uint32_t ex = (uint32_t)(cqx - cpx + 1), ey = (uint32_t)(cqy - cpy + 1), ez = (uint32_t)(cqz - cpz + 1);
     const uint32_t emax = ex > ey ? (ex > ez ? ex : ez) : (ey > ez ? ey : ez);
     const uint32_t bit = (uint32_t)(((cpx & 1) << 4) | ((cpy & 3) << 2) | (cpz & 3));
-    asm volatile("s_waitcnt vmcnt(0)" ::: "memory");
-    uint32_t near_bit = (VL_U(Lay::NEARW + lane) >> bit) & 1u;
+    uint32_t near_bit = (vs.nearw >> bit) & 1u;
     const bool start_free = use_near & (near_bit == 0u);
     const bool need = !first & !((was_in != 0u) & in_q & (emax <= 2u) & start_free);
     VL_I(Lay::CELL + lane) = cqx; VL_I(Lay::CELL + 64 + lane) = cqy; VL_I(Lay::CELL + 128 + lane) = cqz;
     VL_U(Lay::INPREV + lane) = in_q ? 1u : 0u;
     {
-      const uint32_t nb = (uint32_t)h.Nb;
+      const uint32_t nb = vs.nb;
+      const uint64_t *near_grid = vs.near_grid;
       uint32_t w = (((uint32_t)cqx >> 2) * nb + ((uint32_t)cqy >> 2)) * nb + ((uint32_t)cqz >> 2);
-      w = in_q ? 2u * w + (((uint32_t)cqx >> 1) & 1u) : 0u;
+      w = 2u * w + (((uint32_t)cqx >> 1) & 1u);
+      asm volatile("" : "+v"(w));
+      w = in_q ? w : 0u;
       asm volatile("" : "+v"(w) : "v"(near_bit));
       typedef __attribute__((address_space(3))) uint32_t *lds_u32_ptr;
-      __builtin_amdgcn_global_load_lds((const __attribute__((address_space(1))) uint32_t *)h.near_grid + w,
+      __builtin_amdgcn_global_load_lds((const __attribute__((address_space(1))) uint32_t *)near_grid + w,
                                        (lds_u32_ptr)((uint32_t *)vlds + Lay::NEARW), 4, 0, 0);
     }
     return need;
@@ -280,48 +322,53 @@
 
   __device__ __forceinline__ V3 to_voxel_frame(const VerdictArgs &a, const V3 &p) const {
 #pragma clang fp contract(off)
-    if (a.hot.rot_is_identity) return p;
+    if (rot_is_identity()) return p;
     const GridK &g = a.g;
     return V3{g.inv_rot[0] * p.x + g.inv_rot[1] * p.y + g.inv_rot[2] * p.z, g.inv_rot[3] * p.x + g.inv_rot[4] * p.y + g.inv_rot[5] * p.z,
               g.inv_rot[6] * p.x + g.inv_rot[7] * p.y + g.inv_rot[8] * p.z};
   }
 
-  __device__ __forceinline__ void operator()(int j, double x, double y, double z) {
+  __device__ __forceinline__ void operator()(int j, double x, double y, double z, int ms) {
 #pragma clang fp contract(off)
     VL_BARRIER();
-    const VerdictArgs &a = args();
-    const GridK &g = a.g;
+    if constexpr (!SPH) request_landed();
     const int lane = threadIdx.x;
+    const bool first = j == 0;
     const V3 q = {x, y, z};
-    V3 pv = q;
-    float d = 0.0f;
-    if (j > 0) { pv = V3{VL_D(lane), VL_D(64 + lane), VL_D(128 + lane)}; d = VL_F(Lay::DIST + lane); }
+    V3 pv = V3{VL_D(Lay::PREV + lane), VL_D(Lay::PREV + 64 + lane), VL_D(Lay::PREV + 128 + lane)};
+    float d = VL_F(Lay::DIST + lane);
+    const uint32_t hit_before = VL_U(Lay::HIT + lane);
+    HotBox hb;
+    if constexpr (!SPH) hb = hot_box();
+    pv.x = first ? q.x : pv.x; pv.y = first ? q.y : pv.y; pv.z = first ? q.z : pv.z; d = first ? 0.0f : d;
     {
       const float dx = (float)(q.x - pv.x), dy = (float)(q.y - pv.y), dz = (float)(q.z - pv.z);
       d += __builtin_amdgcn_sqrtf(dx * dx + dy * dy + dz * dz);
+    }
+    auto leave = [&]() {
       VL_F(Lay::DIST + lane) = d;
-    }
-    if (j == ms_next) {
-      const int CH_ = a.hot.CH, P_ = a.hot.P;
-      const int o = Lay::MS + ms_k * 64 + lane, pl = a.NM * 64;
-      VL_F(o) = (float)q.x; VL_F(o + pl) = (float)q.y; VL_F(o + 2 * pl) = (float)q.z; VL_F(o + 3 * pl) = d;
-      ms_next = (ms_next + CH_ < P_ - 1) ? ms_next + CH_ : P_ - 1;
-      ms_k++;
-    }
-    VL_D(lane) = q.x; VL_D(64 + lane) = q.y; VL_D(128 + lane) = q.z;
+      if (ms >= 0) {
+        const int o = Lay::MS + ms * 64 + lane, pl = hot_word(kHotMsPlaneW);
+        VL_F(o) = (float)q.x; VL_F(o + pl) = (float)q.y; VL_F(o + 2 * pl) = (float)q.z; VL_F(o + 3 * pl) = d;
+      }
+      VL_D(Lay::PREV + lane) = q.x; VL_D(Lay::PREV + 64 + lane) = q.y; VL_D(Lay::PREV + 128 + lane) = q.z;
+    };
+    if constexpr (SPH) leave();
     bool need = false;
     V3 pr = pv, qr = q;
     bool in_q = false;
     int cq[3] = {0, 0, 0};
     if constexpr (!SPH) {
       double tq[3];
-      point_cell(a, q, qr, in_q, cq, tq);
-      if constexpr (SIG) sig_put(a, j, true, signature_of(a, in_q, cq, tq, x, y, z), sig_own_row(), 0);
+      point_cell(hb, q, qr, in_q, cq, tq);
+      if constexpr (SIG) { const VerdictArgs &a = args(); sig_put(a, j, true, signature_of(a, in_q, cq, tq, x, y, z), sig_own_row(), 0); }
+      need = voxel_test(voxel_state(), first, in_q, cq) & (hit_before == 0u);
+      leave();
     } else {
+      const VerdictArgs &a = args();
+      const GridK &g = a.g;
       if constexpr (SIG) sig_put(a, j, true, cell_signature(x, y, z, g), sig_own_row(), 0);
-    }
-    if constexpr (SPH) {
-      if (active && !VL_U(Lay::HIT + lane)) {
+      if (active && !hit_before) {
         if (sph_state & 1u) {
           if (!g.rot_is_identity) {
             pr.x = g.inv_rot[0] * pv.x + g.inv_rot[1] * pv.y + g.inv_rot[2] * pv.z;
@@ -336,12 +383,11 @@
         sph_state = 0;
         if (!VL_U(Lay::HIT + lane)) request(a, q);
       }
-    } else
-    if (active && !VL_U(Lay::HIT + lane)) need = voxel_test(a.hot, j == 0, in_q, cq);
+    }
     const unsigned long long wm = __ballot(need);
     if (wm) {
       if (need) {
-        if constexpr (!SPH) pr = to_voxel_frame(a, pv);
+        if constexpr (!SPH) pr = to_voxel_frame(args(), pv);
         const int slot = Lay::wrap(qhead + qcount + __popcll(wm & (((unsigned long long)1 << lane) - 1)));
         VL_D(Lay::QE + 0 * VQ + slot) = pr.x; VL_D(Lay::QE + 1 * VQ + slot) = pr.y; VL_D(Lay::QE + 2 * VQ + slot) = pr.z;
         if constexpr (!SPH) { VL_D(Lay::QE + 3 * VQ + slot) = qr.x; VL_D(Lay::QE + 4 * VQ + slot) = qr.y; VL_D(Lay::QE + 5 * VQ + slot) = qr.z; }
@@ -366,7 +412,7 @@
     bool in_q = false;
     int cq[3] = {0, 0, 0};
     double tq[3] = {0.0, 0.0, 0.0};
-    if constexpr (!SPH) point_cell(a, q, qr, in_q, cq, tq);
+    if constexpr (!SPH) point_cell(hot_box(), q, qr, in_q, cq, tq);
     if constexpr (SIG) {
       uint32_t sg = 0u;
       if constexpr (!SPH) sg = on ? signature_of(a, in_q, cq, tq, x, y, z) : 0u;
@@ -378,7 +424,7 @@
     }
     if (on) {
       float d = 0.0f;
-      if (!first) { pv = V3{VL_D(lane), VL_D(64 + lane), VL_D(128 + lane)}; d = VL_F(Lay::DIST + lane); }
+      if (!first) { pv = V3{VL_D(Lay::PREV + lane), VL_D(Lay::PREV + 64 + lane), VL_D(Lay::PREV + 128 + lane)}; d = VL_F(Lay::DIST + lane); }
       pr = pv;
       {
         const float dx = (float)(q.x - pv.x), dy = (float)(q.y - pv.y), dz = (float)(q.z - pv.z);
@@ -395,7 +441,7 @@
           VL_F(o) = (float)q.x; VL_F(o + pl) = (float)q.y; VL_F(o + 2 * pl) = (float)q.z; VL_F(o + 3 * pl) = -d;
         }
       }
-      VL_D(lane) = q.x; VL_D(64 + lane) = q.y; VL_D(128 + lane) = q.z;
+      VL_D(Lay::PREV + lane) = q.x; VL_D(Lay::PREV + 64 + lane) = q.y; VL_D(Lay::PREV + 128 + lane) = q.z;
       if constexpr (SPH) {
         if (active && !VL_U(Lay::HIT + lane)) {
           if (sph_state & 1u) {
@@ -413,7 +459,7 @@
           if (!VL_U(Lay::HIT + lane)) request(a, q);
         }
       } else
-      if (active && !VL_U(Lay::HIT + lane)) need = voxel_test(a.hot, first, in_q, cq);
+      if (active && !VL_U(Lay::HIT + lane)) { request_landed(); need = voxel_test(voxel_state(), first, in_q, cq); }
     }
     const unsigned long long wm = __ballot(need);
     if (wm) {
@@ -478,22 +524,15 @@
 #ifndef TRK_VERDICT_TWO_WAVE_MAXN
 #define TRK_VERDICT_TWO_WAVE_MAXN 4
 #endif
-template <int N, bool ROT, bool SPH, bool SIG = false, class Form = TableRouting>
+template <int N, bool ROT, bool SPH, bool SIG = false, class Form = TableRouting, bool FAST = false>
 __global__ __launch_bounds__(64, (N <= TRK_VERDICT_TWO_WAVE_MAXN ? 2 : 1)) void fk_verdict(
     const double *__restrict__ states, int64_t n, RobotK K, const double *__restrict__ tab, const StepK *__restrict__ steps,
     int nsteps, double *__restrict__ tips, const VerdictArgs *__restrict__ va) {
   using Lay = VLay<SIG>;
   const int lane = threadIdx.x;
-  PointSweep<SPH, SIG> ps;
-  ps.va = va;
-  ps.dn_prev = 0.0f; ps.sph_state = 0u;
-  ps.qhead = 0; ps.qcount = 0; ps.active = false;
-  ps.P = va->P; ps.CH = va->CH; ps.NM = va->NM; ps.Kl = (ps.P - 1 + ps.CH - 1) / ps.CH; ps.ms_next = 0; ps.ms_k = 0;
-  VL_U(Lay::HIT + lane) = 0u; VL_U(Lay::INPREV + lane) = 0u; VL_F(Lay::DIST + lane) = 0.0f;
-  {
-    const int64_t i0 = (int64_t)blockIdx.x * 64 + lane;
-    ps.sigst.init(); ps.sig_row_of = -1; ps.sig_first_row = 0; ps.sig_rows_of_launch(n);
-  }
+  PointSweep<SPH, SIG, FAST> ps;
+  ps.init(va);
+  ps.sig_rows_of_launch(n);
   __syncthreads();
 
   FkLane<N> fl_;
@@ -505,13 +544,13 @@
   while (ps.qcount > 0) ps.flush();
   __syncthreads();
   if (tips) {
-    VL_D(lane) = fl_.tip[0]; VL_D(64 + lane) = fl_.tip[1]; VL_D(128 + lane) = fl_.tip[2];
+    VL_D(Lay::PREV + lane) = fl_.tip[0]; VL_D(Lay::PREV + 64 + lane) = fl_.tip[1]; VL_D(Lay::PREV + 128 + lane) = fl_.tip[2];
     __syncthreads();
     const int64_t e0 = (int64_t)blockIdx.x * 192, etot = 3 * n;
 #pragma unroll
     for (int q = 0; q < 3; q++) {
       const int e = q * 64 + lane;
-      if (e0 + e < etot) tips[e0 + e] = VL_D((e % 3) * 64 + e / 3);
+      if (e0 + e < etot) tips[e0 + e] = VL_D(Lay::PREV + (e % 3) * 64 + e / 3);
     }
     __syncthreads();
   }
@@ -542,16 +581,13 @@
   using Lay = VLay<SIG>;
   const int lane = threadIdx.x;
   PointSweep<SPH, SIG> ps;
-  ps.va = va;
-  ps.dn_prev = 0.0f; ps.sph_state = 0u;
-  ps.qhead = 0; ps.qcount = 0; ps.active = false;
-  ps.P = va->P; ps.CH = va->CH; ps.NM = va->NM; ps.Kl = 0; ps.ms_next = 0; ps.ms_k = 0;
+  ps.init(va);
+  ps.Kl = 0;
   const int32_t *__restrict__ perm = va->perm;
   {
     const int64_t i0 = (int64_t)blockIdx.x * 64 + lane;
-    ps.sigst.init(); ps.sig_row_of = i0 < n ? (perm ? perm[i0] : (int)i0) : -1; ps.sig_first_row = 0; ps.sig_row0 = 0; ps.sig_cnt = 0;
-  }
-  VL_U(Lay::HIT + lane) = 0u; VL_U(Lay::INPREV + lane) = 0u; VL_F(Lay::DIST + lane) = 0.0f;
+    ps.sig_row_of = i0 < n ? (perm ? perm[i0] : (int)i0) : -1;
+  }
   __syncthreads();
 
   FkLaneR<N> fl_;
diff --git a/interactive-rate-tendons_amd/engine.py b/interactive-rate-tendons_amd/engine.py
--- a/interactive-rate-tendons_amd/engine.py
+++ b/interactive-rate-tendons_amd/engine.py
@@ -187,6 +187,11 @@
     def set_debug(self, bits):
         L.check(self._ctx, self.lib.tr_set_debug(self._ctx, int(bits)))
 
+    def verdict_hook_last(self):
+        v = C.c_int32(-1)
+        L.check(self._ctx, self.lib.tr_verdict_hook_last(self._ctx, C.byref(v)))
+        return int(v.value)
+
     def edge_schedule_last(self):
         st = (C.c_uint32 * 4)()
         L.check(self._ctx, self.lib.tr_edge_schedule_last(self._ctx, st))
diff --git a/profiles/count_isa.py b/profiles/count_isa.py
--- a/profiles/count_isa.py
+++ b/profiles/count_isa.py
@@ -51,13 +51,13 @@
 #include <hip/hip_runtime.h>
 #include "tr_types.hpp"
 #include "verdict_kernel.hpp"
-template __global__ void trk::fk_verdict<3, false, false>(const double*, int64_t, RobotK, const double*, const StepK*, int, double*, const trk::VerdictArgs*);
+template __global__ void trk::fk_verdict<3, false, false, false, trk::TableRouting, true>(const double*, int64_t, RobotK, const double*, const StepK*, int, double*, const trk::VerdictArgs*);
 ''',
     "fk_verdict<4,false>": r'''
 #include <hip/hip_runtime.h>
 #include "tr_types.hpp"
 #include "verdict_kernel.hpp"
-template __global__ void trk::fk_verdict<4, false, false>(const double*, int64_t, RobotK, const double*, const StepK*, int, double*, const trk::VerdictArgs*);
+template __global__ void trk::fk_verdict<4, false, false, false, trk::TableRouting, true>(const double*, int64_t, RobotK, const double*, const StepK*, int, double*, const trk::VerdictArgs*);
 ''',
     "fk_sweep_fused<3,false>": r'''
 #include <hip/hip_runtime.h>
@@ -93,7 +93,7 @@
 #include <hip/hip_runtime.h>
 #include "tr_types.hpp"
 #include "verdict_kernel.hpp"
-template __global__ void trk::fk_verdict<3, false, false, false, trk::UniformHelix>(const double*, int64_t, RobotK, const double*, const StepK*, int, double*, const trk::VerdictArgs*);
+template __global__ void trk::fk_verdict<3, false, false, false, trk::UniformHelix, true>(const double*, int64_t, RobotK, const double*, const StepK*, int, double*, const trk::VerdictArgs*);
 ''',
     "fk_sweep_fused_helix<3,false>": r'''
 #include <hip/hip_runtime.h>
diff --git a/profiles/kbench.hip b/profiles/kbench.hip
--- a/profiles/kbench.hip
+++ b/profiles/kbench.hip
@@ -12,6 +12,11 @@
 constexpr bool kSig = true;
 #else
 constexpr bool kSig = false;
+#endif
+#ifdef KB_GENERIC_HOOK
+constexpr bool kFast = false;
+#else
+constexpr bool kFast = !kSig;
 #endif
 #endif
 
@@ -82,9 +87,10 @@
   routing_at(N, C, D, 0.0, tab.data());
   for (int k = 0; k < 128; k++) {
     const double tk = k * dL;
-    steps.push_back(StepK{dL, k + 1, 0});
+    steps.push_back(StepK{dL, k + 1, -1});
     for (int q = 0; q < 3; q++) routing_at(N, C, D, tk + 0.5 * q * dL, &tab[(size_t)(1 + 3 * k + q) * N * 6]);
   }
+  fill_milestone_slots(steps, 129, (int)std::lround(2.0 * K.radius / dL));
 #ifdef KB_COUNT
   const int64_t n = KB_COUNT;
 #else
@@ -123,7 +129,7 @@
   for (int r = 0; r < KB_REPS + 2; r++) {
     CK(hipEventRecord(a));
 #ifdef KB_VERDICT
-    hipLaunchKernelGGL((trk::fk_verdict<N, false, false, kSig, KbForm>), dim3((unsigned)((n + 63) / 64)), dim3(64), lds, nullptr, d_st, n, K, d_tab, d_steps, 128, d_tips, d_va);
+    hipLaunchKernelGGL((trk::fk_verdict<N, false, false, kSig, KbForm, kFast>), dim3((unsigned)((n + 63) / 64)), dim3(64), lds, nullptr, d_st, n, K, d_tab, d_steps, 128, d_tips, d_va);
 #else
     hipLaunchKernelGGL((trk::rk4_only<N>), dim3((unsigned)((n + 63) / 64)), dim3(64), 0, nullptr, d_st, n, K, d_tab, d_steps, 128, d_tips);
 #endif
@@ -137,7 +143,7 @@
   std::sort(ms.begin(), ms.end());
   hipFuncAttributes fa;
 #ifdef KB_VERDICT
-  CK(hipFuncGetAttributes(&fa, (const void *)trk::fk_verdict<N, false, false, kSig, KbForm>));
+  CK(hipFuncGetAttributes(&fa, (const void *)trk::fk_verdict<N, false, false, kSig, KbForm, kFast>));
   {
     std::vector<uint64_t> bits((size_t)((n + 63) / 64));
     CK(hipMemcpy(bits.data(), d_bits, bits.size() * 8, hipMemcpyDeviceToHost));
```

Result: no change. 136.5 million, median of 5 (+0.6%).
